# arnaucube/go-snark-study

Measured on AMD Instinct MI355X. Metric: Groth16 constraints/sec (prove) at 2^20 R1CS, higher is better.
Workload: dtype u32 (9x29-bit Montgomery limbs of the 254-bit BN128 fields)

## Files before the change

### go-snark-study_amd/capi.py

```python
import ctypes
import os
import threading

import numpy as np

_HERE = os.path.dirname(os.path.abspath(__file__))
_LIB = None
_LOCK = threading.Lock()
_INIT_DEVICE = None

u64p = ctypes.POINTER(ctypes.c_uint64)
u32p = ctypes.POINTER(ctypes.c_uint32)
intp = ctypes.POINTER(ctypes.c_int)
Handle = ctypes.c_uint64


class GosnarkHipError(RuntimeError):
    def __init__(self, code, msg):
        super().__init__("libgosnark_hip: status %d: %s" % (code, msg))
        self.code = code


class Timing(ctypes.Structure):
    _fields_ = ([(n, ctypes.c_float) for n in
                 ("total_ms", "plan_ms", "accumulate_ms", "reduce_ms", "poly_ms", "h2d_ms", "acc_g1_ms", "acc_g2_ms")]
                + [("acc_g1_launches", ctypes.c_uint32), ("acc_g2_launches", ctypes.c_uint32),
                   ("acc_g1_terms", ctypes.c_uint64), ("acc_g2_terms", ctypes.c_uint64),
                   ("acc_g1_adds", ctypes.c_uint64), ("acc_g2_adds", ctypes.c_uint64),
                   ("window_bits", ctypes.c_uint32), ("fallbacks", ctypes.c_uint32),
                   ("plan_digits", ctypes.c_uint64), ("plan_entries", ctypes.c_uint64), ("heavy_buckets", ctypes.c_uint32), ("reserved", ctypes.c_uint32)])


class Memory(ctypes.Structure):
    _fields_ = [(n, ctypes.c_uint64) for n in ("device_total_bytes", "device_free_bytes", "library_bytes", "object_bytes", "table_bytes",
                                               "workspace_bytes", "objects", "evictions")]


def lib_path():
    return os.environ.get("GS_LIB") or os.path.join(_HERE, "libgosnark_hip.so")


_SIGS = {
    "gs_init": [intp, ctypes.c_int],
    "gs_free": [Handle],
    "gs_len": [Handle, ctypes.POINTER(ctypes.c_size_t)],
    "gs_g1_upload": [u64p, ctypes.c_size_t, ctypes.POINTER(Handle)],
    "gs_g2_upload": [u64p, ctypes.c_size_t, ctypes.POINTER(Handle)],
    "gs_g1_download": [Handle, u64p, ctypes.c_size_t],
    "gs_g2_download": [Handle, u64p, ctypes.c_size_t],
    "gs_g1_fixed_base": [u64p, ctypes.c_size_t, ctypes.POINTER(Handle)],
    "gs_g2_fixed_base": [u64p, ctypes.c_size_t, ctypes.POINTER(Handle)],
    "gs_scalars_upload": [u64p, ctypes.c_size_t, ctypes.POINTER(Handle)],
    "gs_scalars_download": [Handle, u64p, ctypes.c_size_t],
    "gs_scalars_update": [Handle, u64p, ctypes.c_size_t],
    "gs_msm_g1": [Handle, u64p, ctypes.c_size_t, ctypes.c_size_t, u64p, intp],
    "gs_msm_g2": [Handle, u64p, ctypes.c_size_t, ctypes.c_size_t, u64p, intp],
    "gs_msm_g1_resident": [Handle, ctypes.c_size_t, Handle, ctypes.c_size_t, ctypes.c_size_t, u64p, intp],
    "gs_msm_g2_resident": [Handle, ctypes.c_size_t, Handle, ctypes.c_size_t, ctypes.c_size_t, u64p, intp],
    "gs_msm_g1_begin": [Handle, ctypes.c_size_t, Handle, ctypes.c_size_t, ctypes.c_size_t, u64p],
    "gs_msm_g2_begin": [Handle, ctypes.c_size_t, Handle, ctypes.c_size_t, ctypes.c_size_t, u64p],
    "gs_msm_end": [ctypes.c_uint64, u64p, intp],
    "gs_g1_sum_affine": [u64p, intp, ctypes.c_size_t, u64p, intp],
    "gs_g2_sum_affine": [u64p, intp, ctypes.c_size_t, u64p, intp],
    "gs_poly_mul": [u64p, ctypes.c_size_t, u64p, ctypes.c_size_t, u64p],
    "gs_poly_div": [u64p, ctypes.c_size_t, u64p, ctypes.c_size_t, u64p, u64p],
    "gs_poly_add": [u64p, ctypes.c_size_t, u64p, ctypes.c_size_t, u64p],
    "gs_poly_sub": [u64p, ctypes.c_size_t, u64p, ctypes.c_size_t, u64p],
    "gs_poly_eval": [u64p, ctypes.c_size_t, u64p, u64p],
    "gs_lagrange_interpolation": [u64p, ctypes.c_size_t, u64p],
    "gs_zpoly": [ctypes.c_size_t, u64p],
    "gs_r1cs_to_px": [ctypes.c_size_t, ctypes.c_size_t, u32p, u32p, u64p, u32p, u32p, u64p, u32p, u32p, u64p,
                      u64p, u64p, u64p, u64p, u64p],
    "gs_r1cs_upload": [ctypes.c_size_t, ctypes.c_size_t, u32p, u32p, u64p, u32p, u32p, u64p, u32p, u32p, u64p, ctypes.POINTER(Handle)],
    "gs_r1cs_px": [Handle, Handle, ctypes.POINTER(Handle)],
    "gs_groth16_pk_create": [Handle, Handle, Handle, Handle, Handle, u64p, u64p, u64p, u64p, u64p,
                             u64p, ctypes.c_size_t, ctypes.c_size_t, ctypes.c_size_t, ctypes.POINTER(Handle)],
    "gs_groth16_prove": [Handle, u64p, ctypes.c_size_t, u64p, ctypes.c_size_t, u64p, u64p, u64p, intp],
    "gs_groth16_prove_resident": [Handle, Handle, Handle, u64p, u64p, u64p, intp],
    "gs_groth16_prove_r1cs": [Handle, Handle, Handle, ctypes.POINTER(Handle), u64p, u64p, u64p, intp],
    "gs_groth16_prove_witness": [Handle, Handle, Handle, u64p, u64p, u64p, intp],
    "gs_groth16_prove_witness_begin": [Handle, Handle, Handle, u64p, u64p, u64p],
    "gs_groth16_pk_set_eval": [Handle, Handle],
    "gs_pk_eval_count": [Handle, ctypes.POINTER(ctypes.c_size_t)],
    "gs_pinocchio_pk_set_eval": [Handle, Handle],
    "gs_pinocchio_prove_witness_begin": [Handle, Handle, Handle, u64p],
    "gs_groth16_prove_begin": [Handle, Handle, Handle, u64p, u64p, u64p],
    "gs_groth16_prove_end": [ctypes.c_uint64, u64p, intp],
    "gs_groth16_prove_host_begin": [Handle, u64p, ctypes.c_size_t, u64p, ctypes.c_size_t, u64p, u64p, u64p],
    "gs_groth16_prove_witness_host_begin": [Handle, Handle, u64p, ctypes.c_size_t, u64p, u64p, u64p],
    "gs_groth16_prove_witness_host": [Handle, Handle, u64p, ctypes.c_size_t, u64p, u64p, u64p, intp],
    "gs_pinocchio_prove_host_begin": [Handle, u64p, ctypes.c_size_t, u64p, ctypes.c_size_t, u64p],
    "gs_pinocchio_prove_witness_host_begin": [Handle, Handle, u64p, ctypes.c_size_t, u64p],
    "gs_pinocchio_prove_witness_host": [Handle, Handle, u64p, ctypes.c_size_t, u64p, intp],
    "gs_ticket_cancel": [ctypes.c_uint64],
    "gs_groth16_pk_create_shard": [Handle, Handle, Handle, Handle, Handle, u64p, u64p, u64p, u64p, u64p, u64p, ctypes.c_size_t,
                                   ctypes.c_size_t, ctypes.c_size_t, ctypes.c_size_t, ctypes.c_size_t, ctypes.c_size_t, ctypes.POINTER(Handle)],
    "gs_groth16_pk_shard": [Handle, ctypes.c_size_t, ctypes.c_size_t, ctypes.POINTER(Handle)],
    "gs_groth16_prove_partials": [Handle, Handle, Handle, ctypes.c_size_t, ctypes.c_size_t, u64p, intp],
    "gs_groth16_finish": [Handle, u64p, intp, u64p, u64p, u64p, intp],
    "gs_groth16_setup": [ctypes.c_size_t, ctypes.c_size_t, ctypes.c_size_t, u32p, u32p, u64p, u32p, u32p, u64p, u32p, u32p, u64p,
                         u64p, ctypes.POINTER(Handle), u64p],
    "gs_groth16_pk_export": [Handle, ctypes.c_int, u64p, ctypes.c_size_t],
    "gs_pinocchio_setup": [ctypes.c_size_t, ctypes.c_size_t, ctypes.c_size_t, u32p, u32p, u64p, u32p, u32p, u64p, u32p, u32p, u64p,
                           u64p, ctypes.POINTER(Handle), u64p],
    "gs_pinocchio_pk_export": [Handle, ctypes.c_int, u64p, ctypes.c_size_t],
    "gs_pinocchio_pk_create": [Handle, Handle, Handle, Handle, Handle, Handle, Handle, Handle, u64p,
                               ctypes.c_size_t, ctypes.c_size_t, ctypes.c_size_t, ctypes.POINTER(Handle)],
    "gs_pinocchio_prove": [Handle, u64p, ctypes.c_size_t, u64p, ctypes.c_size_t, u64p, intp],
    "gs_pinocchio_prove_resident": [Handle, Handle, Handle, u64p, intp],
    "gs_pinocchio_prove_witness": [Handle, Handle, Handle, u64p, intp],
    "gs_pinocchio_prove_begin": [Handle, Handle, Handle, u64p],
    "gs_pinocchio_prove_end": [ctypes.c_uint64, u64p, intp],
    "gs_device_count": [],
    "gs_set_device": [ctypes.c_int],
    "gs_get_device": [],
    "gs_handle_device": [Handle],
    "gs_scalars_clone": [Handle, ctypes.c_size_t, ctypes.c_size_t, ctypes.c_int, ctypes.POINTER(Handle)],
    "gs_g1_clone": [Handle, ctypes.c_size_t, ctypes.c_size_t, ctypes.c_int, ctypes.POINTER(Handle)],
    "gs_g2_clone": [Handle, ctypes.c_size_t, ctypes.c_size_t, ctypes.c_int, ctypes.POINTER(Handle)],
    "gs_groth16_pk_shard_to": [Handle, ctypes.c_size_t, ctypes.c_size_t, ctypes.c_int, ctypes.POINTER(Handle)],
    "gs_comm_unique_id": [ctypes.POINTER(ctypes.c_uint8)],
    "gs_comm_init_rank": [ctypes.POINTER(ctypes.c_uint8), ctypes.c_int, ctypes.c_int],
    "gs_comm_init_local": [],
    "gs_comm_info": [intp, intp, intp, u64p],
    "gs_comm_allgather": [ctypes.c_void_p, ctypes.c_size_t, ctypes.c_void_p],
    "gs_msm_g1_multi": [ctypes.POINTER(Handle), ctypes.POINTER(Handle), ctypes.c_int, u64p, intp, intp],
    "gs_msm_g2_multi": [ctypes.POINTER(Handle), ctypes.POINTER(Handle), ctypes.c_int, u64p, intp, intp],
    "gs_groth16_prove_multi": [ctypes.POINTER(Handle), ctypes.POINTER(Handle), ctypes.POINTER(Handle), ctypes.c_int, u64p, u64p, u64p, intp, intp],
    "gs_groth16_prove_sharded": [Handle, Handle, Handle, u64p, u64p, u64p, intp],
    "gs_groth16_witness_values": [Handle, Handle, Handle, ctypes.POINTER(Handle), ctypes.POINTER(ctypes.c_uint32)],
    "gs_groth16_prove_partials_values": [Handle, Handle, Handle, ctypes.c_size_t, ctypes.c_size_t, u64p, intp],
    "gs_groth16_partials_values_begin": [Handle, Handle, Handle, ctypes.c_size_t, ctypes.c_size_t, u64p],
    "gs_groth16_partials_end": [ctypes.c_uint64, u64p, intp],
    "gs_groth16_prove_multi_values": [ctypes.POINTER(Handle), ctypes.POINTER(Handle), ctypes.POINTER(Handle), ctypes.c_int, u64p, u64p, u64p, intp, intp],
    "gs_groth16_prove_sharded_values": [Handle, Handle, Handle, u64p, u64p, u64p, intp],
    "gs_scalars_scatter": [Handle, ctypes.c_size_t, ctypes.c_int, ctypes.POINTER(Handle)],
    "gs_msm_g1_sharded": [Handle, Handle, u64p, intp],
    "gs_msm_g2_sharded": [Handle, Handle, u64p, intp],
    "gs_groth16_prove_batch": [ctypes.POINTER(Handle), ctypes.c_int, ctypes.POINTER(Handle), ctypes.POINTER(Handle), ctypes.c_size_t,
                               u64p, u64p, u64p, intp],
    "gs_pinocchio_pk_shard": [Handle, ctypes.c_size_t, ctypes.c_size_t, ctypes.POINTER(Handle)],
    "gs_pinocchio_pk_shard_to": [Handle, ctypes.c_size_t, ctypes.c_size_t, ctypes.c_int, ctypes.POINTER(Handle)],
    "gs_pinocchio_prove_partials": [Handle, Handle, Handle, ctypes.c_size_t, ctypes.c_size_t, u64p, intp],
    "gs_pinocchio_witness_values": [Handle, Handle, Handle, ctypes.POINTER(Handle), ctypes.POINTER(ctypes.c_uint32)],
    "gs_pinocchio_prove_partials_values": [Handle, Handle, Handle, ctypes.c_size_t, ctypes.c_size_t, u64p, intp],
    "gs_pinocchio_combine": [u64p, intp, ctypes.c_size_t, u64p, intp],
    "gs_pinocchio_prove_multi": [ctypes.POINTER(Handle), ctypes.POINTER(Handle), ctypes.POINTER(Handle), ctypes.c_int, u64p, intp, intp],
    "gs_pinocchio_prove_multi_values": [ctypes.POINTER(Handle), ctypes.POINTER(Handle), ctypes.POINTER(Handle), ctypes.c_int, u64p, intp, intp],
    "gs_pinocchio_prove_sharded": [Handle, Handle, Handle, u64p, intp],
    "gs_pinocchio_prove_sharded_values": [Handle, Handle, Handle, u64p, intp],
    "gs_pinocchio_prove_batch": [ctypes.POINTER(Handle), ctypes.c_int, ctypes.POINTER(Handle), ctypes.POINTER(Handle), ctypes.c_size_t, u64p, intp],
    "gs_last_timing": [ctypes.POINTER(Timing)],
    "gs_device_timing": [ctypes.c_int, ctypes.POINTER(Timing)],
    "gs_set_window_bits": [ctypes.c_int],
    "gs_set_eval_basis": [ctypes.c_int],
    "gs_memory_query": [ctypes.POINTER(Memory)],
    "gs_handle_bytes": [Handle, u64p, u64p],
    "gs_release_tables": [Handle],
    "gs_set_table_policy": [ctypes.c_int],
    "gs_build_tables": [Handle, ctypes.c_int],
    "gs_set_memory_limit": [ctypes.c_uint64],
    "gs_alloc_counters": [u64p, u64p],
    "gs_abi_sizes": [ctypes.POINTER(ctypes.c_size_t), ctypes.POINTER(ctypes.c_size_t)],
    "gs_trim": [],
    "gs_verify_set_strict": [ctypes.c_int],
    "gs_pairing": [u64p, u64p, u64p],
    "gs_pairing_check": [u64p, u64p, ctypes.c_size_t, intp],
    "gs_groth16_verify": [u64p, u64p, u64p, u64p, u64p, ctypes.c_size_t, u64p, ctypes.c_size_t, u64p, u64p, u64p, intp],
    "gs_pinocchio_verify": [u64p, u64p, u64p, u64p, u64p, u64p, u64p, u64p, ctypes.c_size_t, u64p, ctypes.c_size_t, u64p, intp, intp],
}
EXPORTS = sorted(list(_SIGS) + ["gs_shutdown", "gs_last_error", "gs_version", "gs_comm_destroy"])


def load_library():
    global _LIB
    with _LOCK:
        if _LIB is not None:
            return _LIB
        path = lib_path()
        try:
            import torch
        except ImportError:
            pass
        if not os.path.exists(path):
            raise GosnarkHipError(-1, "%s not found: build it with __graft_entry__.build() "
                                  "(hipcc --offload-arch=gfx950); there is no CPU fallback" % path)
        lib = ctypes.CDLL(path)
        missing = [n for n in EXPORTS if not hasattr(lib, n)]
        if missing:
            raise GosnarkHipError(-1, "%s lacks symbols declared in include/gosnark_hip.h: %s" % (path, missing))
        for name, args in _SIGS.items():
            fn = getattr(lib, name)
            fn.argtypes = args
            fn.restype = ctypes.c_int
        lib.gs_last_error.restype = ctypes.c_char_p
        lib.gs_version.restype = ctypes.c_char_p
        lib.gs_shutdown.restype = None
        lib.gs_comm_destroy.restype = None
        tb, mb = ctypes.c_size_t(0), ctypes.c_size_t(0)
        lib.gs_abi_sizes(ctypes.byref(tb), ctypes.byref(mb))
        if tb.value != ctypes.sizeof(Timing) or mb.value != ctypes.sizeof(Memory):
            raise GosnarkHipError(-1, "%s writes gs_timing / gs_memory of %d / %d bytes, this binding expects %d / %d: rebuild the library"
                                  % (path, tb.value, mb.value, ctypes.sizeof(Timing), ctypes.sizeof(Memory)))
        _LIB = lib
        return lib


def check(status):
# ... 219 lines not shown
def memory_query():
    init()
    m = Memory()
    check(load_library().gs_memory_query(ctypes.byref(m)))
    return {n: int(getattr(m, n)) for n, _ in Memory._fields_ if n != "reserved"}


def handle_bytes(h):
    a, b = ctypes.c_uint64(0), ctypes.c_uint64(0)
    check(load_library().gs_handle_bytes(Handle(_raw(h)), ctypes.cast(ctypes.byref(a), u64p), ctypes.cast(ctypes.byref(b), u64p)))
    return int(a.value), int(b.value)


def release_tables(h):
    check(load_library().gs_release_tables(Handle(_raw(h))))


TABLE_POLICY = {"auto": 0, "always": 1, "never": 2}


def set_table_policy(policy):
    init()
    check(load_library().gs_set_table_policy(TABLE_POLICY[policy] if isinstance(policy, str) else int(policy)))


def build_tables(h, route=0):
    check(load_library().gs_build_tables(Handle(_raw(h)), int(route)))


def set_memory_limit(nbytes):
    check(load_library().gs_set_memory_limit(ctypes.c_uint64(int(nbytes))))


def alloc_counters():
    a, b = ctypes.c_uint64(0), ctypes.c_uint64(0)
    check(load_library().gs_alloc_counters(ctypes.cast(ctypes.byref(a), u64p), ctypes.cast(ctypes.byref(b), u64p)))
    return int(a.value), int(b.value)


def scalars_update(handle, s_u64):
    a = np.ascontiguousarray(s_u64, dtype=np.uint64).reshape(-1, 4)
    check(load_library().gs_scalars_update(Handle(_raw(handle)), ptr64(a), a.shape[0]))


def trim():
    check(load_library().gs_trim())


def set_eval_basis(on):
    init()
    check(load_library().gs_set_eval_basis(1 if on else 0))


def set_window_bits(c):
    init()
    check(load_library().gs_set_window_bits(int(c)))


def zpoly(deg):
    init()
    out = np.zeros((deg + 1, 4), dtype=np.uint64)
    check(load_library().gs_zpoly(deg, ptr64(out)))
    return out


def msm_begin(bases, scalars, n, off=0, soff=0, g2=False):
    t = ctypes.c_uint64(0)
    fn = load_library().gs_msm_g2_begin if g2 else load_library().gs_msm_g1_begin
    check(fn(Handle(bases.h), off, Handle(scalars.h), soff, n, ctypes.cast(ctypes.byref(t), u64p)))
    return (t.value, g2)


def ticket_cancel(ticket):
    check(load_library().gs_ticket_cancel(ctypes.c_uint64(ticket[0] if isinstance(ticket, tuple) else ticket)))


def msm_end(ticket):
    t, g2 = ticket
    out = np.zeros(16 if g2 else 8, dtype=np.uint64)
    inf = ctypes.c_int(0)
    check(load_library().gs_msm_end(ctypes.c_uint64(t), ptr64(out), ctypes.byref(inf)))
    return _affine_result(out, inf, g2)


def _clone(fname, handle, off, n, target):
    h = Handle(0)
    check(getattr(load_library(), fname)(Handle(handle.h), off, n, int(target), ctypes.byref(h)))
    return DeviceHandle(h.value)


def scalars_clone(handle, target, off=0, n=None):
    return _clone("gs_scalars_clone", handle, off, len(handle) - off if n is None else n, target)


def g1_clone(handle, target, off=0, n=None):
    return _clone("gs_g1_clone", handle, off, len(handle) - off if n is None else n, target)


def g2_clone(handle, target, off=0, n=None):
    return _clone("gs_g2_clone", handle, off, len(handle) - off if n is None else n, target)


def scalars_scatter(full_handle, total, root, slice_handle=None):
    h = Handle(slice_handle.h if slice_handle is not None else 0)
    check(load_library().gs_scalars_scatter(Handle(full_handle.h if full_handle is not None else 0), int(total), int(root), ctypes.byref(h)))
    return slice_handle if slice_handle is not None else DeviceHandle(h.value)
# ... 60 lines not shown
```

### go-snark-study_amd/csrc/capi_msm.hip

```cpp
#include <algorithm>
#include <cstdlib>
#include <vector>

#include "msm.h"
#include "hostcopy.h"
#include "point_io.h"
#include "poly.h"
#include "prove.h"
#include "runtime.h"

using namespace gs;

namespace gs { void multi_shutdown(); }

namespace {


template <class T>
int upload_bases(Ctx& c, Kind kind, const uint64_t* jac, size_t n, gs_handle* out) {
  if (!out || (n && !jac)) return fail(GS_ERR_ARG, "null argument");
  if (n >= (1ull << 31)) return fail(GS_ERR_ARG, "too many points");
  constexpr size_t cw = T::kWords;
  auto b = std::make_unique<Bases>(kind);
  b->n = n;
// ... 500 lines not shown
  return guarded([&](Ctx& c) -> int {
    if (!out) return fail(GS_ERR_ARG, "null");
    *out = c.timing;
    return GS_OK;
  }, true, true);
}

int gs_device_timing(int logical_device, gs_timing* out) {
  if (!out) return fail(GS_ERR_ARG, "null");
  std::shared_ptr<Ctx> pc = ctx_ref(logical_device);
  if (!pc) return fail(GS_ERR_ARG, "gs_device_timing: no logical device %d", logical_device);
  Ctx& c = *pc;
  std::lock_guard<FairMutex> lk(c.mu);
  if (!c.ready) return fail(GS_ERR_NOT_INIT, "the library was shut down");
  *out = c.timing;
  return GS_OK;
}

int gs_ticket_cancel(uint64_t ticket) {
  return guarded([&](Ctx& c) -> int {
    for (int p = 0; p < Ctx::kMaxInFlight; ++p)
      if (c.inflight[p] && c.inflight[p]->ticket == ticket) {
        c.drain();
        c.inflight[p].reset();
        return GS_OK;
      }
    return fail(GS_ERR_ARG, "gs_ticket_cancel: unknown ticket %llu", (unsigned long long)ticket);
  }, true, true, ticket);
}

int gs_set_window_bits(int cbits) {
  if (cbits != 0 && (cbits < 8 || cbits > kMaxWindowBits)) return fail(GS_ERR_ARG, "window bits must be 0 (auto) or 8..%d", kMaxWindowBits);
  Registry& r = registry();
  std::lock_guard<std::mutex> rl(r.mu);
  if (r.ctxs.empty()) return fail(GS_ERR_NOT_INIT, "gs_init has not been called (or failed)");
  for (auto& pc : r.ctxs) {
    std::lock_guard<FairMutex> lk(pc->mu);
    pc->window_bits = cbits;
  }
  return GS_OK;
}

int gs_set_eval_basis(int enabled) {
  Registry& r = registry();
  std::lock_guard<std::mutex> rl(r.mu);
  if (r.ctxs.empty()) return fail(GS_ERR_NOT_INIT, "gs_init has not been called (or failed)");
  for (auto& pc : r.ctxs) {
    std::lock_guard<FairMutex> lk(pc->mu);
    pc->eval_basis = enabled != 0;
  }
  return GS_OK;
}

}
```

### go-snark-study_amd/csrc/capi_poly.hip

```cpp
#include "prove.h"

#include <algorithm>

using namespace gs;

extern "C" {

int gs_poly_mul(const uint64_t* a, size_t na, const uint64_t* b, size_t nb, uint64_t* out) {
  return guarded([&](Ctx& c) -> int {
    if (!a || !b || !out || na == 0 || nb == 0) return fail(GS_ERR_ARG, "gs_poly_mul: empty or null operand");
    if (na + nb > (1ull << 27)) return fail(GS_ERR_ARG, "gs_poly_mul: product too large");
    const uint32_t* da = upload_tmp(c, prove_state(c).up_a, a, na);
    const uint32_t* db = upload_tmp(c, prove_state(c).up_b, b, nb);
    const size_t nr = na + nb - 1;
    prove_state(c).up_o.ensure(nr * 32);
    poly_mul_dev(c, da, na, Form::Std, db, nb, Form::Std, prove_state(c).up_o.as<uint32_t>());
    poly_canon_dev(c, prove_state(c).up_o.as<uint32_t>(), nr, 0);
    download(c, out, prove_state(c).up_o.p, nr);
    return GS_OK;
  });
}

int gs_poly_div(const uint64_t* a, size_t na, const uint64_t* b, size_t nb, uint64_t* quo, uint64_t* rem) {
  return guarded([&](Ctx& c) -> int {
    if (!a || !b || !quo || nb == 0 || na < nb) return fail(GS_ERR_ARG, "gs_poly_div: need len(a) >= len(b) >= 1");
    bool lead_zero = true;
    for (int i = 0; i < 4; ++i) lead_zero = lead_zero && b[4 * (nb - 1) + i] == 0;
    if (lead_zero) return fail(GS_ERR_ARG, "gs_poly_div: leading coefficient of the divisor is zero");
    const uint32_t* da = upload_tmp(c, prove_state(c).up_a, a, na);
    const uint32_t* db = upload_tmp(c, prove_state(c).up_b, b, nb);
    Divisor d;
    divisor_init(c, d, db, nb);
    const size_t nq = na - nb + 1;
    prove_state(c).up_o.ensure((nq + na + nb) * 32);
    uint32_t* q = prove_state(c).up_o.as<uint32_t>();
    poly_quotient_dev(c, d, da, na, q);
    if (rem && nb > 1) {
      uint32_t* qb = q + nq * 8;
      poly_mul_dev(c, q, nq, Form::Std, db, nb, Form::Std, qb);
      uint32_t* rr = qb + (nq + nb - 1) * 8;
      poly_addsub_dev(c, da, nb - 1, qb, nb - 1, true, rr);
      poly_canon_dev(c, rr, nb - 1, 0);
      GS_HIP(hipMemcpyAsync(rem, rr, (nb - 1) * 32, hipMemcpyDeviceToHost, c.stream));
      GS_HIP(hipStreamSynchronize(c.stream));
    }
    poly_canon_dev(c, q, nq, 0);
    download(c, quo, q, nq);
    return GS_OK;
  });
}

static int addsub_api(const uint64_t* a, size_t na, const uint64_t* b, size_t nb, uint64_t* out, bool sub) {
  return guarded([&](Ctx& c) -> int {
    if ((na && !a) || (nb && !b) || !out) return fail(GS_ERR_ARG, "null operand");
    const size_t n = std::max(na, nb);
    if (n == 0) return GS_OK;
    const uint32_t* da = upload_tmp(c, prove_state(c).up_a, a, na);
    const uint32_t* db = upload_tmp(c, prove_state(c).up_b, b, nb);
    prove_state(c).up_o.ensure(n * 32);
    poly_addsub_dev(c, da, na, db, nb, sub, prove_state(c).up_o.as<uint32_t>());
    poly_canon_dev(c, prove_state(c).up_o.as<uint32_t>(), n, 0);
    download(c, out, prove_state(c).up_o.p, n);
    return GS_OK;
  });
}
int gs_poly_add(const uint64_t* a, size_t na, const uint64_t* b, size_t nb, uint64_t* out) { return addsub_api(a, na, b, nb, out, false); }
int gs_poly_sub(const uint64_t* a, size_t na, const uint64_t* b, size_t nb, uint64_t* out) { return addsub_api(a, na, b, nb, out, true); }

int gs_poly_eval(const uint64_t* v, size_t n, const uint64_t x[4], uint64_t out[4]) {
  return guarded([&](Ctx& c) -> int {
    if ((n && !v) || !x || !out) return fail(GS_ERR_ARG, "null operand");
    const uint32_t* dv = upload_tmp(c, prove_state(c).up_a, v, n);
    prove_state(c).up_o.ensure(32);
    poly_eval_dev(c, dv, n, x, prove_state(c).up_o.as<uint32_t>());
    download(c, out, prove_state(c).up_o.p, 1);
    return GS_OK;
  });
}

int gs_lagrange_interpolation(const uint64_t* values, size_t n, uint64_t* coeffs) {
  return guarded([&](Ctx& c) -> int {
    if (n == 0) return GS_OK;
    if (!values || !coeffs) return fail(GS_ERR_ARG, "gs_lagrange_interpolation: null argument");
    if (n >= (1ull << 26)) return fail(GS_ERR_ARG, "gs_lagrange_interpolation: too many nodes");
    const uint32_t* dv = upload_tmp(c, prove_state(c).up_a, values, n);
    prove_state(c).up_o.ensure(n * 32);
    interpolate_dev(c, dv, n, 1, prove_state(c).up_o.as<uint32_t>());
    poly_canon_dev(c, prove_state(c).up_o.as<uint32_t>(), n, 0);
    download(c, coeffs, prove_state(c).up_o.p, n);
    return GS_OK;
  });
}

int gs_zpoly(size_t deg, uint64_t* out) {
  return guarded([&](Ctx& c) -> int {
    if (!out) return fail(GS_ERR_ARG, "gs_zpoly: null output");
    if (deg >= (1ull << 26)) return fail(GS_ERR_ARG, "gs_zpoly: degree too large");
    prove_state(c).up_o.ensure((deg + 1) * 32);
    zpoly_dev(c, deg, prove_state(c).up_o.as<uint32_t>());
    download(c, out, prove_state(c).up_o.p, deg + 1);
// ... 6 lines not shown
```

### go-snark-study_amd/csrc/msm.hip

```cpp
#include "msm.h"
#include "hostcopy.h"

#include <algorithm>
#include <cmath>
#include <cstdlib>
#include <future>
#include <type_traits>

#include "msm_kernels.h"

namespace gs {

static_assert(sizeof(G1Xyzz) == PointIO<FqTag>::kXyzzWords * 4, "G1 XYZZ must be raw limbs");
static_assert(sizeof(G2Xyzz) == PointIO<Fq2Tag>::kXyzzWords * 4, "G2 XYZZ must be raw limbs");

static inline dim3 grid1(size_t n, int block = 256) { return dim3((unsigned)((n + block - 1) / block)); }

int choose_window_bits(uint32_t n, int forced) {
  if (forced >= 8 && forced <= kMaxWindowBits) return forced;
  static const double per_bucket = dev_knob_f("GS_WINDOW_COST_BUCKET", 6.0, 0.0, 64.0);
  static const int auto_max = (int)dev_knob("GS_AUTO_MAX_C", 17, 8, kMaxWindowBits);
  int best = 8;
  double best_cost = 1e300;
  for (int c = 8; c <= std::min(kMaxWindowBits, std::max(8, auto_max)); ++c) {
// ... 36 lines not shown
};
static MsmState& msm_state(Ctx& c) { return c.state<MsmState>(c.msm_state); }

static uint32_t choose_chunk(uint64_t entries, uint32_t nbuckets, const std::vector<LaunchShape>& users) {
  static const int forced = (int)dev_knob("GS_CHUNK", 0, 4, 1024, 4);
  if (forced >= 4 && forced % 4 == 0) return (uint32_t)forced;
  static const int forced_h = (int)dev_knob("GS_CHUNK_H", 0, 4, 1024, 4);
  if (forced_h && users.size() == 1 && users[0].njobs == 1 && !users[0].g2) return (uint32_t)forced_h;
  uint32_t chunk = entries >= (1ull << 27) ? 64u : entries >= (1ull << 23) ? 32u : 16u;
  while (chunk < 1024u && entries / std::max<uint32_t>(nbuckets, 1u) > 32ull * chunk) chunk *= 2;
  return chunk;
}

static uint32_t part_min_ranges() {
  static const uint32_t v = (uint32_t)dev_knob("GS_PART_MIN_R", 4, 2, 64);
  return v;
}
bool plan_partitions_first(int cbits) {
  if (cbits < 1) return false;
  return std::max<uint32_t>(1u, (1u << (cbits - 1)) >> kRangeLog) >= part_min_ranges();
}

uint32_t finite_mask_dev(Ctx& c, const uint32_t* g1_pts, const uint32_t* g2_pts, uint32_t n, uint32_t* mask_dev) {
  const size_t words = ((size_t)n + 31) / 32;
  GS_HIP(hipMemsetAsync(mask_dev, 0, std::max<size_t>(words, 1) * 4, c.stream));
  DevBuf cnt(4);
  GS_HIP(hipMemsetAsync(cnt.p, 0, 4, c.stream));
  if (n) hipLaunchKernelGGL(k_finite_mask, grid1(n), dim3(256), 0, c.stream, g1_pts, (uint32_t)PointIO<FqTag>::kAffineWords, g2_pts,
                            (uint32_t)PointIO<Fq2Tag>::kAffineWords, n, mask_dev, cnt.as<uint32_t>());
  GS_HIP(hipGetLastError());
  uint32_t host = 0;
  GS_HIP(hipMemcpyAsync(&host, cnt.p, 4, hipMemcpyDeviceToHost, c.stream));
  GS_HIP(hipStreamSynchronize(c.stream));
  return host;
}

void build_plan(Ctx& c, int slot, const uint32_t* scalars_dev, uint32_t n, MsmPlan& plan, const std::vector<LaunchShape>& users, int cbits,
                bool table_free, const uint32_t* term_index, uint32_t index_bias) {
  MsmState& ms = msm_state(c);
  PlanBuffers& pb = ms.plan_slots[slot % (3 * Ctx::kSlots)];
  plan.n = n;
  plan.table_free = table_free;
  plan.c = cbits ? cbits : (table_free ? choose_window_bits_free(n, c.window_bits) : choose_window_bits(n, c.window_bits));
  if (table_free && (plan.c < kMinFreeWindowBits || plan.c > kMaxFreeWindowBits))
    throw HipError{hipErrorInvalidValue, "table-free plan outside 9..16 window bits", __LINE__};
  plan.W = 254 / plan.c + 1;
  plan.B = 1u << (plan.c - 1);
  plan.nbuckets = table_free ? (uint32_t)plan.W * plan.B : plan.B;
  plan.chunk = choose_chunk((uint64_t)n * plan.W, plan.nbuckets, users);
  plan.maxchunks = (uint32_t)(((size_t)n * plan.W + plan.chunk - 1) / plan.chunk) + 1;
  const size_t ncount = (size_t)plan.nbuckets + 1;
  PlanParams pp{};
  pp.n = n; pp.c = plan.c; pp.W = plan.W; pp.B = plan.B;
  pp.R = std::max<uint32_t>(1u, plan.B >> kRangeLog);
  pp.tf = table_free ? 1u : 0u;
  {
    const uint32_t want = std::max<uint32_t>(1u, 256u / (plan.W * pp.R));
    const uint32_t by_size = std::max<uint32_t>(1u, (n + 16383u) / 16384u);
    const uint32_t by_mem = std::max<uint32_t>(1u, (uint32_t)((64ull << 20) / ((uint64_t)plan.B * plan.W * 4)));
    pp.S = std::max<uint32_t>(1u, std::min(std::min<uint32_t>(16u, std::max<uint32_t>(want, 1u)), std::min(by_size, by_mem)));
    if (pp.R == 1 && !table_free) pp.S = std::max<uint32_t>(1u, std::min<uint32_t>(16u, by_size));
  }
  pp.slice = (n + pp.S - 1) / pp.S;
  pp.stride = (n + 63u) & ~63u;
  const bool wide = plan_partitions_first(plan.c);
  if (wide && term_index) throw HipError{hipErrorInvalidValue, "plans over a term list cannot be sorted partition-first (plan_partitions_first)", __LINE__};
  const uint32_t nparts = (uint32_t)plan.W * pp.R;
  if (wide && nparts > kMaxParts) throw HipError{hipErrorInvalidValue, "too many (window, range) partitions", __LINE__};
  if (!wide) pb.digits.ensure((size_t)std::max<uint32_t>(pp.stride, 64u) * plan.W * sizeof(digit_t));
  else {
    pb.recs.ensure(std::max<size_t>((size_t)n * plan.W, 1) * 8);
    pb.parts.ensure((size_t)(3 * kMaxParts + 4) * 4);
  }
  pb.hist.ensure((size_t)plan.B * plan.W * pp.S * 4);
  pb.totals.ensure(ncount * 4);
  pb.offsets.ensure(ncount * 4);
  pb.entries.ensure(((size_t)plan.maxchunks + 1) * plan.chunk * 4);
  pb.chunk_bucket.ensure((size_t)plan.maxchunks * 4);
  pb.heavy_list.ensure((size_t)plan.nbuckets * 4);
  pb.counters.ensure(16);
  const size_t lds = (size_t)std::min<uint32_t>(plan.B, kRangeBuckets) * 4;
  static const int sort_block = (int)dev_knob("GS_SORT_BLOCK", kSortBlock, 64, kSortBlock, 64);
  if (!ms.lds_attr_set) {
    GS_HIP(hipFuncSetAttribute(reinterpret_cast<const void*>(k_hist), hipFuncAttributeMaxDynamicSharedMemorySize, 128 * 1024));
    GS_HIP(hipFuncSetAttribute(reinterpret_cast<const void*>(k_scatter), hipFuncAttributeMaxDynamicSharedMemorySize, 128 * 1024));
    GS_HIP(hipFuncSetAttribute(reinterpret_cast<const void*>(k_hist_part), hipFuncAttributeMaxDynamicSharedMemorySize, 128 * 1024));
    GS_HIP(hipFuncSetAttribute(reinterpret_cast<const void*>(k_scatter_part), hipFuncAttributeMaxDynamicSharedMemorySize, 128 * 1024));
    ms.lds_attr_set = true;
  }
  GS_HIP(hipMemsetAsync(pb.totals.as<uint32_t>() + plan.nbuckets, 0, 4, c.stream));
  GS_HIP(hipMemsetAsync(pb.counters.p, 0, 16, c.stream));
  uint32_t* part_count = pb.parts.as<uint32_t>();
  uint32_t* part_base = part_count ? part_count + kMaxParts : nullptr;
  uint32_t* part_cursor = part_count ? part_base + kMaxParts + 4 : nullptr;
  if (n > 0 && wide) {
    GS_HIP(hipMemsetAsync(part_count, 0, (size_t)nparts * 4, c.stream));
    hipLaunchKernelGGL(k_part_count, grid1(n, kPartBlock), dim3(kPartBlock), 0, c.stream, scalars_dev, pp, part_count);
    hipLaunchKernelGGL(k_part_scan, dim3(1), dim3(64), 0, c.stream, part_count, nparts, part_base, part_cursor);
    hipLaunchKernelGGL(k_part_scatter, grid1(n, kPartBlock * kPartPerThread), dim3(kPartBlock), 0, c.stream, scalars_dev, pp, part_base, part_cursor,
                       pb.recs.as<uint2>());
    hipLaunchKernelGGL(k_hist_part, dim3(8 * pp.S * ((nparts + 7) / 8)), dim3(sort_block), lds, c.stream, pb.recs.as<uint2>(), part_base, pp, pb.hist.as<uint32_t>());
    hipLaunchKernelGGL(k_colscan, grid1(plan.B), dim3(256), 0, c.stream, pb.hist.as<uint32_t>(), pp, pb.totals.as<uint32_t>());
  } else if (n > 0) {
    hipLaunchKernelGGL(k_digits, grid1(n), dim3(256), 0, c.stream, scalars_dev, pp, pb.digits.as<digit_t>(), term_index, index_bias);
    hipLaunchKernelGGL(k_hist, dim3(plan.W, pp.S, pp.R), dim3(sort_block), lds, c.stream, pb.digits.as<digit_t>(), pp, pb.hist.as<uint32_t>());
    if (table_free) hipLaunchKernelGGL(k_colscan_windows, grid1(plan.nbuckets), dim3(256), 0, c.stream, pb.hist.as<uint32_t>(), pp, pb.totals.as<uint32_t>());
    else hipLaunchKernelGGL(k_colscan, grid1(plan.B), dim3(256), 0, c.stream, pb.hist.as<uint32_t>(), pp, pb.totals.as<uint32_t>());
  } else {
    GS_HIP(hipMemsetAsync(pb.totals.p, 0, ncount * 4, c.stream));
  }
  exclusive_scan(c, pb, pb.totals.as<uint32_t>(), pb.offsets.as<uint32_t>(), (uint32_t)ncount);
  if (n > 0) {
    if (wide) hipLaunchKernelGGL(k_scatter_part, dim3(8 * pp.S * ((nparts + 7) / 8)), dim3(sort_block), lds, c.stream, pb.recs.as<uint2>(), part_base, pp,
                                 pb.hist.as<uint32_t>(), pb.offsets.as<uint32_t>(), pb.entries.as<uint32_t>());
    else hipLaunchKernelGGL(k_scatter, dim3(plan.W, pp.S, pp.R), dim3(sort_block), lds, c.stream, pb.digits.as<digit_t>(), pp, pb.hist.as<uint32_t>(),
                            pb.offsets.as<uint32_t>(), pb.entries.as<uint32_t>(), term_index, index_bias);
    hipLaunchKernelGGL(k_chunk_map, grid1(plan.nbuckets), dim3(256), 0, c.stream, pb.offsets.as<uint32_t>(), plan.nbuckets, plan.chunk,
                       pb.chunk_bucket.as<uint32_t>(), pb.heavy_list.as<uint32_t>(), pb.counters.as<uint32_t>());
  }
  GS_HIP(hipGetLastError());
  plan.offsets = pb.offsets.as<uint32_t>();
  plan.entries = pb.entries.as<uint32_t>();
  plan.chunk_bucket = pb.chunk_bucket.as<uint32_t>();
  plan.heavy_list = pb.heavy_list.as<uint32_t>();
  plan.heavy_count = pb.counters.as<uint32_t>();
}

template <class T>
static void enqueue_table_slabs(hipStream_t stream, DevBuf& scratch, const uint32_t* src, size_t n, int cbits, DevBuf& rows, size_t first, size_t last,
                                size_t slab) {
  const int W = 254 / cbits + 1;
  if (first >= last) return;
  static const bool per_row = dev_flag("GS_TABLE_PER_ROW");
  if (per_row || W <= 2) {
    if (first == 0) hipLaunchKernelGGL(k_build_table<T>, grid1(n), dim3(256), 0, stream, src, (uint32_t)n, cbits, W, rows.as<uint32_t>());
  } else {
    constexpr size_t sw = PointIO<T>::kXyzzWords + PointIO<T>::kXyzzWords / 4;
    slab = std::min<size_t>(std::max<size_t>(slab, 1), n);
    scratch.ensure(slab * (size_t)(W - 1) * sw * 4);
    for (size_t at = first; at < last; at += slab) {
      const size_t count = std::min(slab, last - at);
      hipLaunchKernelGGL(k_build_table_batched<T>, grid1(count), dim3(256), 0, stream, src, (uint32_t)n, (uint32_t)at, (uint32_t)count, cbits, W,
                         rows.as<uint32_t>(), scratch.as<uint32_t>());
    }
  }
  GS_HIP(hipGetLastError());
}
template <class T>
static void enqueue_table_build(Ctx& c, hipStream_t stream, DevBuf& scratch, const uint32_t* src, size_t n, int cbits, DevBuf& fresh,
                                size_t slab_max = (size_t)1 << 18) {
  constexpr size_t aw = PointIO<T>::kAffineWords;
  const int W = 254 / cbits + 1;
  fresh.alloc(std::max<size_t>(n, 1) * W * aw * 4);
  enqueue_table_slabs<T>(stream, scratch, src, n, cbits, fresh, 0, n, slab_max);
}

template <class T>
static void ensure_table(Ctx& c, BaseTable& t, const uint32_t* row0, size_t n, int cbits) {
  if (t.c == cbits && t.n == n && t.rows.p) return;
  table_settle(c, t, false);
  const uint32_t* src = row0 ? row0 : t.rows.as<uint32_t>();
  if (!src || (!row0 && t.n != n)) throw HipError{hipErrorInvalidValue, "window table rebuild without its points", __LINE__};
  DevBuf fresh;
  enqueue_table_build<T>(c, c.stream, msm_state(c).table_scratch, src, n, cbits, fresh);
  GS_HIP(hipStreamSynchronize(c.stream));
  t.rows = std::move(fresh);
  t.n = n; t.c = cbits; t.W = 254 / cbits + 1;
  t.uses = 0;
// ... 457 lines not shown
```

### go-snark-study_amd/csrc/msm_kernels.h

```cpp
#pragma once
#include <hip/hip_runtime.h>
#include <stdint.h>

#include "ec.h"
#include "point_io.h"

namespace gs {

struct PlanParams {
  uint32_t n;
  int c;
  int W;
  uint32_t B;
  uint32_t S;
  uint32_t slice;
  uint32_t stride;
  uint32_t R;
  uint32_t tf;
};
constexpr uint32_t kRangeLog = 15;
constexpr uint32_t kRangeBuckets = 1u << kRangeLog;

GS_HD int32_t next_digit(const uint32_t (&k)[8], const PlanParams& pp, int w, uint32_t& carry) {
  uint32_t raw = scalar_bits(k, w * pp.c, pp.c) + carry;
  if (raw > pp.B) { carry = 1; return (int32_t)raw - (int32_t)(2u * pp.B); }
  carry = 0;
  return (int32_t)raw;
}

using digit_t = uint32_t;
__global__ void __launch_bounds__(256) k_digits(const uint32_t* __restrict__ scalars, PlanParams pp, digit_t* __restrict__ digits,
                                                 const uint32_t* __restrict__ term_index, uint32_t index_bias) {
  wave_priority<GS_PRIO_PLAN>();
  const uint32_t i = blockIdx.x * blockDim.x + threadIdx.x;
  if (i >= pp.n) return;
  const uint32_t src = term_index ? term_index[i] - index_bias : i;
  uint32_t k[8];
  const uint4* s4 = reinterpret_cast<const uint4*>(scalars + (size_t)src * 8);
  uint4 lo = s4[0], hi = s4[1];
  k[0] = lo.x; k[1] = lo.y; k[2] = lo.z; k[3] = lo.w; k[4] = hi.x; k[5] = hi.y; k[6] = hi.z; k[7] = hi.w;
  scalar_canon(k);
  uint32_t carry = 0;
  for (int w = 0; w < pp.W; ++w) {
    const int32_t d = next_digit(k, pp, w, carry);
    digits[(size_t)w * pp.stride + i] = (digit_t)(d + (int32_t)pp.B - 1);
  }
}

__global__ void __launch_bounds__(256) k_finite_mask(const uint32_t* __restrict__ a, uint32_t wa, const uint32_t* __restrict__ b, uint32_t wb, uint32_t n,
                                                      uint32_t* __restrict__ mask, uint32_t* __restrict__ count) {
  const uint32_t i = blockIdx.x * blockDim.x + threadIdx.x;
  bool finite = false;
  if (i < n) {
    uint32_t acc = 0;
    if (a) for (uint32_t k = 0; k < wa; ++k) acc |= a[(size_t)i * wa + k];
    if (b) for (uint32_t k = 0; k < wb; ++k) acc |= b[(size_t)i * wb + k];
    finite = acc != 0;
  }
  if (finite) { atomicOr(&mask[i >> 5], 1u << (i & 31u)); atomicAdd(count, 1u); }
}

constexpr int kSortBlock = 1024;

__global__ void __launch_bounds__(kSortBlock) k_hist(const digit_t* __restrict__ digits, PlanParams pp, uint32_t* __restrict__ hist) {
  wave_priority<GS_PRIO_PLAN>();
  extern __shared__ uint32_t sh[];
  const uint32_t w = blockIdx.x, s = blockIdx.y, r = blockIdx.z;
  const uint32_t nb = min(pp.B, kRangeBuckets), base = r << kRangeLog;
  for (uint32_t b = threadIdx.x; b < nb; b += blockDim.x) sh[b] = 0;
  __syncthreads();
  const uint32_t lo = s * pp.slice, hi = min(pp.n, lo + pp.slice);
  const digit_t* row = digits + (size_t)w * pp.stride;
  const int32_t zero = (int32_t)pp.B - 1;
  for (uint32_t i = lo + threadIdx.x; i < hi; i += blockDim.x) {
    const int32_t d = (int32_t)row[i] - zero;
    if (d != 0) {
      const uint32_t b = (uint32_t)(d < 0 ? -d : d) - 1u;
      if ((b >> kRangeLog) == r) atomicAdd(&sh[b - base], 1u);
    }
  }
  __syncthreads();
  uint32_t* out = hist + ((size_t)w * pp.S + s) * pp.B + base;
  for (uint32_t b = threadIdx.x; b < nb; b += blockDim.x) out[b] = sh[b];
}

__global__ void __launch_bounds__(256) k_colscan(uint32_t* __restrict__ hist, PlanParams pp, uint32_t* __restrict__ totals) {
  wave_priority<GS_PRIO_PLAN>();
  const uint32_t b = blockIdx.x * blockDim.x + threadIdx.x;
  if (b >= pp.B) return;
  uint32_t* col = hist + b;
  const uint32_t nq = (uint32_t)pp.W * pp.S;
  uint32_t run = 0;
  for (uint32_t q = 0; q < nq; ++q) { const uint32_t t = col[(size_t)q * pp.B]; col[(size_t)q * pp.B] = run; run += t; }
  totals[b] = run;
}

__global__ void __launch_bounds__(256) k_colscan_windows(uint32_t* __restrict__ hist, PlanParams pp, uint32_t* __restrict__ totals) {
  wave_priority<GS_PRIO_PLAN>();
  const uint32_t i = blockIdx.x * blockDim.x + threadIdx.x;
  if (i >= (uint32_t)pp.W * pp.B) return;
  const uint32_t w = i / pp.B, b = i % pp.B;
  uint32_t* col = hist + (size_t)w * pp.S * pp.B + b;
  uint32_t run = 0;
  for (uint32_t q = 0; q < pp.S; ++q) { const uint32_t t = col[(size_t)q * pp.B]; col[(size_t)q * pp.B] = run; run += t; }
  totals[i] = run;
}

__global__ void __launch_bounds__(kSortBlock) k_scatter(const digit_t* __restrict__ digits, PlanParams pp, const uint32_t* __restrict__ hist,
                                                         const uint32_t* __restrict__ offsets, uint32_t* __restrict__ entries,
                                                         const uint32_t* __restrict__ term_index, uint32_t index_bias) {
  wave_priority<GS_PRIO_PLAN>();
  extern __shared__ uint32_t sh[];
  const uint32_t w = blockIdx.x, s = blockIdx.y, r = blockIdx.z;
  const uint32_t nb = min(pp.B, kRangeBuckets), base = r << kRangeLog;
  const uint32_t* pre = hist + ((size_t)w * pp.S + s) * pp.B + base;
  const uint32_t* off = offsets + (pp.tf ? (size_t)w * pp.B : (size_t)0);
  for (uint32_t b = threadIdx.x; b < nb; b += blockDim.x) sh[b] = off[base + b] + pre[b];
  __syncthreads();
  const uint32_t lo = s * pp.slice, hi = min(pp.n, lo + pp.slice);
  const digit_t* row = digits + (size_t)w * pp.stride;
  const int32_t zero = (int32_t)pp.B - 1;
  for (uint32_t i = lo + threadIdx.x; i < hi; i += blockDim.x) {
    const int32_t d = (int32_t)row[i] - zero;
    if (d != 0) {
      const uint32_t b = (uint32_t)(d < 0 ? -d : d) - 1u;
      if ((b >> kRangeLog) == r) {
        const uint32_t pos = atomicAdd(&sh[b - base], 1u);
        const uint32_t id = term_index ? term_index[i] - index_bias : i;
        entries[pos] = id | (w << kWindowShift) | (d < 0 ? kSignBit : 0u);
      }
    }
  }
}

constexpr int kPartBlock = 256;
constexpr int kPartPerThread = 4;
constexpr uint32_t kMaxParts = 512;

GS_HD void load_scalar_canon(const uint32_t* __restrict__ scalars, uint32_t i, uint32_t (&k)[8]) {
  const uint4* s4 = reinterpret_cast<const uint4*>(scalars + (size_t)i * 8);
  const uint4 lo = s4[0], hi = s4[1];
  k[0] = lo.x; k[1] = lo.y; k[2] = lo.z; k[3] = lo.w; k[4] = hi.x; k[5] = hi.y; k[6] = hi.z; k[7] = hi.w;
  scalar_canon(k);
}

__global__ void __launch_bounds__(kPartBlock) k_part_count(const uint32_t* __restrict__ scalars, PlanParams pp, uint32_t* __restrict__ part_count) {
  wave_priority<GS_PRIO_PLAN>();
  __shared__ uint32_t cnt[kMaxParts];
  const uint32_t nparts = (uint32_t)pp.W * pp.R;
  for (uint32_t t = threadIdx.x; t < nparts; t += kPartBlock) cnt[t] = 0;
  __syncthreads();
  const uint32_t i = blockIdx.x * kPartBlock + threadIdx.x;
  if (i < pp.n) {
    uint32_t k[8];
    load_scalar_canon(scalars, i, k);
    uint32_t carry = 0;
    for (int w = 0; w < pp.W; ++w) {
      const int32_t d = next_digit(k, pp, w, carry);
      if (d != 0) atomicAdd(&cnt[(uint32_t)w * pp.R + (((uint32_t)(d < 0 ? -d : d) - 1u) >> kRangeLog)], 1u);
    }
  }
  __syncthreads();
  for (uint32_t t = threadIdx.x; t < nparts; t += kPartBlock) if (cnt[t]) atomicAdd(&part_count[t], cnt[t]);
}

__global__ void __launch_bounds__(64) k_part_scan(uint32_t* __restrict__ part_count, uint32_t nparts, uint32_t* __restrict__ part_base,
                                                    uint32_t* __restrict__ part_cursor) {
  wave_priority<GS_PRIO_PLAN>();
  if (blockIdx.x != 0 || threadIdx.x != 0) return;
  uint32_t run = 0;
  for (uint32_t t = 0; t < nparts; ++t) { part_base[t] = run; run += part_count[t]; part_cursor[t] = 0; part_count[t] = 0; }
  part_base[nparts] = run;
}

__global__ void __launch_bounds__(kPartBlock) k_part_scatter(const uint32_t* __restrict__ scalars, PlanParams pp, const uint32_t* __restrict__ part_base,
                                                              uint32_t* __restrict__ part_cursor, uint2* __restrict__ recs) {
  wave_priority<GS_PRIO_PLAN>();
  __shared__ uint32_t cnt[kMaxParts];
  const uint32_t nparts = (uint32_t)pp.W * pp.R;
  for (uint32_t t = threadIdx.x; t < nparts; t += kPartBlock) cnt[t] = 0;
// ... 628 lines not shown
```

### go-snark-study_amd/csrc/poly.h

```cpp
#pragma once
#include "fp29.h"
#include "runtime.h"

namespace gs {

enum class Form { Std, Mont };

int ceil_log2(size_t n);

void ntt_forward(Ctx& c, uint32_t* data, int logt, int logm);
void ntt_inverse_unscaled(Ctx& c, uint32_t* data, int logt, int logm);
void ntt_forward_n(Ctx& c, uint32_t* data, size_t total, int logm);
void ntt_inverse_unscaled_n(Ctx& c, uint32_t* data, size_t total, int logm);

void poly_mul_dev(Ctx& c, const uint32_t* a, size_t na, Form fa, const uint32_t* b, size_t nb, Form fb, uint32_t* out);

void poly_inv_series_dev(Ctx& c, const uint32_t* f_mont, size_t nf, size_t k, uint32_t* g_mont);

struct Divisor {
  size_t nb = 0;
  DevBuf b_std;
  size_t k = 0;
  DevBuf inv_rev_mont;
  int logn_spec = 0;
  size_t k_spec = 0;
  DevBuf inv_spec;
};
void divisor_init(Ctx& c, Divisor& d, const uint32_t* b_std_dev, size_t nb);
void poly_quotient_dev(Ctx& c, Divisor& d, const uint32_t* a_std, size_t na, uint32_t* quo_std);

void zpoly_dev(Ctx& c, size_t deg, uint32_t* out_std);

void interpolate_dev(Ctx& c, const uint32_t* values_std, size_t n, size_t nvec, uint32_t* coeffs_std);
bool hx_direct_dev(Ctx& c, const uint32_t* vals_std, size_t n, size_t dz, uint32_t* hx_out_std);
bool hx_values_dev(Ctx& c, const uint32_t* vals_std, size_t n, size_t dz, uint32_t* hv_out_std);
void r1cs_check_dev(Ctx& c, const uint32_t* vals_std, size_t n, size_t dz, uint32_t* bad_dev);
void hx_from_values_dev(Ctx& c, const uint32_t* hv_std, size_t n, size_t dz, uint32_t* hx_out_std);
void spmv_dev(Ctx& c, const uint32_t* rowptr, const uint32_t* col, const uint32_t* val_std, const uint32_t* x_mont, size_t nrows, size_t ncols,
              uint32_t* out_std);

void poly_addsub_dev(Ctx& c, const uint32_t* a, size_t na, const uint32_t* b, size_t nb, bool subtract, uint32_t* out);
void poly_canon_dev(Ctx& c, uint32_t* x, size_t n, int mode );
void poly_eval_dev(Ctx& c, const uint32_t* v_std, size_t n, const uint64_t x[4], uint32_t* out_dev);

Fe<ModR, 2> fr_from_words_mont(const uint64_t w[4]);
void fr_words_from_mont(const Fe<ModR, 2>& a, uint64_t out[4]);
void fr_mul_words(const uint64_t a[4], const uint64_t b[4], uint64_t out[4]);
void fr_inv_words(const uint64_t a[4], uint64_t out[4]);
void fr_sub_words(const uint64_t a[4], const uint64_t b[4], uint64_t out[4]);
bool fr_is_zero_words(const uint64_t a[4]);
void fr_falling_product_words(const uint64_t x[4], size_t count, uint64_t out[4]);

const uint32_t* interpolation_weights_dev(Ctx& c, size_t n);
void lagrange_at_dev(Ctx& c, size_t n, const uint64_t tau[4], const uint64_t mtau[4], uint32_t* out_mont);
void setup_scalars_dev(Ctx& c, const uint32_t* at, const uint32_t* bt, const uint32_t* ct, size_t m, size_t npublic, const uint64_t kalpha[4],
                       const uint64_t kbeta[4], const uint64_t inv_delta[4], const uint64_t inv_gamma[4], uint32_t* cd, uint32_t* ic);
void pinocchio_scalars_dev(Ctx& c, const uint32_t* at, const uint32_t* bt, const uint32_t* ct, size_t m, const uint64_t rhoa[4], const uint64_t rhob[4],
                           const uint64_t rhoc[4], const uint64_t ka[4], const uint64_t kb[4], const uint64_t kc[4], const uint64_t kbeta[4],
                           uint32_t* const out[7]);
void scaled_powers_dev(Ctx& c, const uint64_t base[4], const uint64_t scale_std[4], size_t count, uint32_t* out_std);
void scale_mont_by_std_dev(Ctx& c, const uint32_t* a_mont, const uint64_t scale_std[4], size_t n, uint32_t* out_std);

}
```

### go-snark-study_amd/csrc/poly.hip

```cpp
#include "poly.h"

#include <algorithm>
#include <vector>

#include "poly_kernels.h"

namespace gs {

static inline dim3 grid1(size_t n, int block = 256) { return dim3((unsigned)((n + block - 1) / block)); }

int ceil_log2(size_t n) {
  int l = 0;
  while (((size_t)1 << l) < n) ++l;
  return l;
}

static FrConst to_const(const Fe<ModR, 2>& a) {
  FrConst c;
  for (int i = 0; i < NL; ++i) c.l[i] = a.l[i];
  return c;
}
Fe<ModR, 2> fr_from_words_mont(const uint64_t w[4]) {
  uint32_t u[8];
  for (int i = 0; i < 4; ++i) { u[2 * i] = (uint32_t)w[i]; u[2 * i + 1] = (uint32_t)(w[i] >> 32); }
  return to_mont(unpack32<ModR>(u));
}
static Fe<ModR, 2> fr_small_mont(uint64_t v) {
  uint64_t w[4] = {v, 0, 0, 0};
  return fr_from_words_mont(w);
}

struct Twiddles {
  int logn = 0;
  DevBuf fwd, inv;
};
struct NodeTree {
  size_t n = 0, total = 0, pad = 0;
  int L = 0;
  std::vector<DevBuf> mspec;
  DevBuf root;
  DevBuf weights;
  uint64_t stamp = 0;
};

struct PolyState {
  Twiddles tw;
  DevBuf ws_a, ws_b, ws_c, ws_d;
  NodeTree trees[2];
  uint64_t tree_clock = 0;
  DevBuf cur_a, cur_b, wide, nxt;
  DevBuf long_rows;
  size_t fact_top = 0;
  DevBuf fact, invfact;
  struct HxTables {
    size_t n = 0, dz = 0, N = 0;
    uint64_t stamp = 0;
    DevBuf inv_spec, shift_spec, t1, t2;
  };
  static constexpr int kHxSlots = 4;
  HxTables hx[kHxSlots];
  uint64_t hx_clock = 0;
  DevBuf hx_conv, hx_hv, hx_g, hx_bad;
};
static PolyState& poly_state(Ctx& c) { return c.state<PolyState>(c.poly_state); }

static Twiddles& ensure_twiddles(Ctx& c, int logn) {
  Twiddles& tw = poly_state(c).tw;
  if (logn <= tw.logn) return tw;
  if (logn > ModR::kTwoAdicity) throw HipError{hipErrorInvalidValue, "NTT size exceeds the 2-adicity of Fr (2^28)", __LINE__};
  logn = std::max(logn, 16);
  const uint32_t half = 1u << (logn - 1);
  Fe<ModR, 2> w, wi;
  for (int i = 0; i < NL; ++i) { w.l[i] = ModR::omega28_mont(i); wi.l[i] = ModR::omega28_inv_mont(i); }
  for (int i = 0; i < ModR::kTwoAdicity - logn; ++i) { w = sqr(w); wi = sqr(wi); }
  tw.fwd.alloc((size_t)half * kTwWords * 4);
  tw.inv.alloc((size_t)half * kTwWords * 4);
  hipLaunchKernelGGL(k_twiddle_gen, grid1(half), dim3(256), 0, c.stream, tw.fwd.as<uint32_t>(), half, to_const(w));
  hipLaunchKernelGGL(k_twiddle_gen, grid1(half), dim3(256), 0, c.stream, tw.inv.as<uint32_t>(), half, to_const(wi));
  GS_HIP(hipGetLastError());
  tw.logn = logn;
  return tw;
}

void ntt_forward(Ctx& c, uint32_t* data, int logt, int logm) { ntt_forward_n(c, data, (size_t)1 << logt, logm); }
void ntt_inverse_unscaled(Ctx& c, uint32_t* data, int logt, int logm) { ntt_inverse_unscaled_n(c, data, (size_t)1 << logt, logm); }

struct NttPass { int s_lo, k, clog; uint32_t ntiles; };
static std::vector<NttPass> ntt_schedule(size_t total, int logm) {
  std::vector<NttPass> v;
  const int low = std::min(kNttMaxStages, logm);
  int hi = logm;
  while (hi > low) {
    const int k = std::min(kNttMaxStages, hi - low);
    const int s_lo = hi - k;
    const int clog = std::min(kNttTileLog - k, s_lo);
    v.push_back(NttPass{s_lo, k, clog, (uint32_t)(total >> (k + clog))});
    hi = s_lo;
  }
  int clog = kNttTileLog - low;
  while (clog > 0 && ((total >> low) & (((size_t)1 << clog) - 1))) --clog;
  v.push_back(NttPass{0, low, clog, (uint32_t)(total >> (low + clog))});
  return v;
}

void ntt_forward_n(Ctx& c, uint32_t* data, size_t total, int logm) {
  if (logm == 0 || total == 0) return;
  Twiddles& tw = ensure_twiddles(c, logm);
  for (const NttPass& p : ntt_schedule(total, logm))
    hipLaunchKernelGGL((k_ntt_pass<false, kNttLoadPlain>), dim3(p.ntiles), dim3(256), 0, c.stream, data, tw.fwd.as<uint32_t>(), tw.logn, p.s_lo, p.k, p.clog, NttLoadAux{});
  GS_HIP(hipGetLastError());
}

void ntt_inverse_unscaled_n(Ctx& c, uint32_t* data, size_t total, int logm) {
  if (logm == 0 || total == 0) return;
  Twiddles& tw = ensure_twiddles(c, logm);
// ... 64 lines not shown
  uint32_t* A = poly_state(c).ws_a.as<uint32_t>();
  uint32_t* B = poly_state(c).ws_b.as<uint32_t>();
  copy_padded(c, a, na, A, N);
  copy_padded(c, b, nb, B, N);
  ntt_forward(c, A, logn, logn);
  ntt_forward(c, B, logn, logn);
  hipLaunchKernelGGL(k_pw_mul, grid1(N), dim3(256), 0, c.stream, A, B, A, (uint32_t)N);
  ntt_inverse_unscaled(c, A, logn, logn);
  hipLaunchKernelGGL(k_pw_mul_const, grid1(nr), dim3(256), 0, c.stream, A, inv_n_const(logn, extra), out, (uint32_t)nr);
  GS_HIP(hipGetLastError());
}

void poly_inv_series_dev(Ctx& c, const uint32_t* f, size_t nf, size_t k, uint32_t* g) {
  Fe<ModR, 6> f0v;
  uint32_t f0w[8];
  GS_HIP(hipMemcpyAsync(f0w, f, 32, hipMemcpyDeviceToHost, c.stream));
  GS_HIP(hipStreamSynchronize(c.stream));
  f0v = unpack32<ModR>(f0w);
  if (is_zero(f0v)) throw HipError{hipErrorInvalidValue, "series inverse of a polynomial with zero constant term", __LINE__};
  Fe<ModR, 2> g0 = inv(reduce2(f0v));
  uint32_t g0w[8];
  {
    Fe<ModR, 1> cg = canon(g0);
    pack32<ModR>(cg, g0w);
  }
  GS_HIP(hipMemcpyAsync(g, g0w, 32, hipMemcpyHostToDevice, c.stream));
  GS_HIP(hipStreamSynchronize(c.stream));
  const FrConst two = to_const(fr_small_mont(2));
  size_t t = 1;
  while (t < k) {
    const size_t t2 = std::min(2 * t, k);
    const size_t fl = std::min(nf, t2);
    poly_state(c).ws_c.ensure((std::max(fl, t2) + t) * 32);
    poly_state(c).ws_d.ensure((t2 + t) * 32);
    uint32_t* E = poly_state(c).ws_c.as<uint32_t>();
    uint32_t* U = poly_state(c).ws_d.as<uint32_t>();
    poly_mul_dev(c, f, fl, Form::Mont, g, t, Form::Mont, E);
    const size_t el = std::min(fl + t - 1, t2);
    hipLaunchKernelGGL(k_two_minus, grid1(t2), dim3(256), 0, c.stream, E, two, U, (uint32_t)el, (uint32_t)t2);
    poly_mul_dev(c, g, t, Form::Mont, U, t2, Form::Mont, E);
    GS_HIP(hipMemcpyAsync(g, E, t2 * 32, hipMemcpyDeviceToDevice, c.stream));
    t = t2;
  }
  GS_HIP(hipGetLastError());
}

void divisor_init(Ctx& c, Divisor& d, const uint32_t* b_std_dev, size_t nb) {
  d.nb = nb;
  d.b_std.alloc(nb * 32);
  GS_HIP(hipMemcpyAsync(d.b_std.p, b_std_dev, nb * 32, hipMemcpyDeviceToDevice, c.stream));
  d.k = 0;
  d.logn_spec = 0;
  d.k_spec = 0;
}

static void divisor_ensure(Ctx& c, Divisor& d, size_t k) {
  if (k <= d.k) return;
  const size_t fl = std::min(d.nb, k);
  DevBuf f(fl * 32);
  hipLaunchKernelGGL(k_copy_reversed, grid1(fl), dim3(256), 0, c.stream, d.b_std.as<uint32_t>(), (uint32_t)(d.nb - fl), (uint32_t)fl,
                     f.as<uint32_t>(), (uint32_t)fl);
  poly_canon_dev(c, f.as<uint32_t>(), fl, 1);
  d.inv_rev_mont.alloc(k * 32);
  poly_inv_series_dev(c, f.as<uint32_t>(), fl, k, d.inv_rev_mont.as<uint32_t>());
  GS_HIP(hipStreamSynchronize(c.stream));
  d.k = k;
  d.logn_spec = 0;
}

void poly_quotient_dev(Ctx& c, Divisor& d, const uint32_t* a, size_t na, uint32_t* quo) {
  if (na < d.nb) return;
  const size_t k = na - d.nb + 1;
  divisor_ensure(c, d, k);
  const int logn = ceil_log2(2 * k - 1);
  const size_t N = (size_t)1 << logn;
  if (d.logn_spec != logn || d.k_spec != k) {
    d.inv_spec.alloc(N * 32);
    copy_padded(c, d.inv_rev_mont.as<uint32_t>(), k, d.inv_spec.as<uint32_t>(), N);
    ntt_forward(c, d.inv_spec.as<uint32_t>(), logn, logn);
    d.logn_spec = logn;
    d.k_spec = k;
  }
  poly_state(c).ws_a.ensure(N * 32);
  uint32_t* A = poly_state(c).ws_a.as<uint32_t>();
  hipLaunchKernelGGL(k_copy_reversed, grid1(N), dim3(256), 0, c.stream, a, (uint32_t)(na - k), (uint32_t)k, A, (uint32_t)N);
  ntt_forward(c, A, logn, logn);
  if (logn >= 1) ntt_inverse_unscaled_of_product_n(c, A, N, logn, d.inv_spec.as<uint32_t>());
  else hipLaunchKernelGGL(k_pw_mul, grid1(N), dim3(256), 0, c.stream, A, d.inv_spec.as<uint32_t>(), A, (uint32_t)N);
  poly_state(c).ws_b.ensure(k * 32);
  hipLaunchKernelGGL(k_copy_reversed, grid1(k), dim3(256), 0, c.stream, A, 0u, (uint32_t)k, poly_state(c).ws_b.as<uint32_t>(), (uint32_t)k);
  hipLaunchKernelGGL(k_pw_mul_const, grid1(k), dim3(256), 0, c.stream, poly_state(c).ws_b.as<uint32_t>(), inv_n_const(logn, 0), quo, (uint32_t)k);
  GS_HIP(hipGetLastError());
}


static void prefix_products(Ctx& c, int mode, uint32_t top, uint32_t count, uint32_t* out, Fe<ModR, 2>* last_host) {
  const uint32_t ntiles = (count + kPpTile - 1) / kPpTile;
  DevBuf tiles((size_t)ntiles * 32);
  hipLaunchKernelGGL(k_pp_tiles, dim3(ntiles), dim3(kPpBlock), 0, c.stream, mode, top, count, out, tiles.as<uint32_t>());
  if (ntiles > 1) {
    hipLaunchKernelGGL(k_pp_tile_scan, dim3(1), dim3(1024), 0, c.stream, tiles.as<uint32_t>(), ntiles);
    hipLaunchKernelGGL(k_pp_apply, grid1(count), dim3(256), 0, c.stream, out, tiles.as<uint32_t>(), count);
  }
  GS_HIP(hipGetLastError());
  if (last_host) {
    uint32_t w[8];
    GS_HIP(hipMemcpyAsync(w, out + (size_t)(count - 1) * 8, 32, hipMemcpyDeviceToHost, c.stream));
    GS_HIP(hipStreamSynchronize(c.stream));
    *last_host = reduce2(unpack32<ModR>(w));
  }
  GS_HIP(hipStreamSynchronize(c.stream));
}
static void ensure_factorials(Ctx& c, size_t top) {
  PolyState& ps = poly_state(c);
  if (top <= ps.fact_top) return;
  top = std::max<size_t>(top, 2 * ps.fact_top);
  if (top >= (1ull << 31)) throw HipError{hipErrorInvalidValue, "factorial table too large", __LINE__};
  DevBuf fwd(top * 32), rev(top * 32);
  Fe<ModR, 2> top_fact;
  prefix_products(c, 0, (uint32_t)top, (uint32_t)top, fwd.as<uint32_t>(), &top_fact);
  prefix_products(c, 1, (uint32_t)top, (uint32_t)top, rev.as<uint32_t>(), nullptr);
  ps.fact.alloc((top + 1) * 32);
  ps.invfact.alloc((top + 1) * 32);
  hipLaunchKernelGGL(k_fact_tables, grid1(top + 1), dim3(256), 0, c.stream, fwd.as<uint32_t>(), rev.as<uint32_t>(), to_const(inv(top_fact)), (uint32_t)top,
                     ps.fact.as<uint32_t>(), ps.invfact.as<uint32_t>());
  GS_HIP(hipGetLastError());
  GS_HIP(hipStreamSynchronize(c.stream));
  ps.fact_top = top;
}

static void build_weights(Ctx& c, NodeTree& t) {
  ensure_factorials(c, std::max<size_t>(t.n, 1));
  t.weights.alloc(std::max<size_t>(t.n, 1) * 32);
  if (t.n) hipLaunchKernelGGL(k_bary_weights, grid1(t.n), dim3(256), 0, c.stream, poly_state(c).invfact.as<uint32_t>(), (uint32_t)t.n, t.weights.as<uint32_t>());
  GS_HIP(hipGetLastError());
  GS_HIP(hipStreamSynchronize(c.stream));
}

static NodeTree& ensure_tree(Ctx& c, size_t n, bool need_weights) {
  NodeTree* t = nullptr;
  PolyState& ps = poly_state(c);
  for (auto& x : ps.trees) if (x.n == n && x.root.p) t = &x;
  if (!t) {
    t = (ps.trees[0].stamp <= ps.trees[1].stamp) ? &ps.trees[0] : &ps.trees[1];
// ... 282 lines not shown
```

### go-snark-study_amd/csrc/poly_kernels.h

```cpp
#pragma once
#include <hip/hip_runtime.h>
#include <stdint.h>

#include "fp29.h"

namespace gs {

using Fr6 = Fe<ModR, 6>;
using Fr2 = Fe<ModR, 2>;

GS_HD Fr6 load_fr(const uint32_t* p) {
  const uint4* q = reinterpret_cast<const uint4*>(p);
  const uint4 lo = q[0], hi = q[1];
  uint32_t w[8] = {lo.x, lo.y, lo.z, lo.w, hi.x, hi.y, hi.z, hi.w};
  return unpack32<ModR>(w);
}
GS_HD void store_fr(uint32_t* p, const Fr2& a) {
  Fr2 x = a;
  carry_full(x);
  Fe<ModR, 1> y;
#pragma unroll
  for (int i = 0; i < NL; ++i) y.l[i] = x.l[i];
  uint32_t w[8];
  pack32<ModR>(y, w);
// ... 88 lines not shown
GS_HD void ntt_dif_butterfly(int step, Bfly (&x)[N], const Fe<ModR, 1> (&w)[N], bool trivial) {
  ntt_dif_step<16, N>(x, w, (step & 3) == 3, trivial);
}
template <int B, int N>
GS_HD void ntt_dit_step(Bfly (&x)[N], const Fe<ModR, 1> (&w)[N], bool lazy_in, bool lazy_out, bool trivial) {
  static_assert(N == 1 || N == 2, "one or two butterflies per thread");
  Fr2 t[N];
  if (trivial) {
#pragma unroll
    for (int k = 0; k < N; ++k)
#pragma unroll
      for (int l = 0; l < NL; ++l) t[k].l[l] = x[k].b[l];
  } else if (lazy_in) {
    Lz<ModR, B, 3> b[N];
#pragma unroll
    for (int k = 0; k < N; ++k)
#pragma unroll
      for (int l = 0; l < NL; ++l) b[k].l[l] = x[k].b[l];
    if constexpr (N == 2) dots2<ModR>(dot_of(b[0], w[0]), dot_of(b[1], w[1]), t[0], t[1]);
    else t[0] = mul_lazy(b[0], w[0]);
  } else {
    Fe<ModR, B> b[N];
#pragma unroll
    for (int k = 0; k < N; ++k)
#pragma unroll
      for (int l = 0; l < NL; ++l) b[k].l[l] = x[k].b[l];
    if constexpr (N == 2) dots2<ModR>(dot_of(b[0], w[0]), dot_of(b[1], w[1]), t[0], t[1]);
    else t[0] = mul_lazy(b[0], w[0]);
  }
#pragma unroll
  for (int k = 0; k < N; ++k) {
    uint32_t p[NL], m[NL];
#pragma unroll
    for (int l = 0; l < NL; ++l) { p[l] = x[k].a[l] + t[k].l[l]; m[l] = x[k].a[l] + (ModR::tbias(3, l) - t[k].l[l]); }
    static_assert(ModR::tbias_k(3) == 3, "the DIT bound table (B + 2, B + 3) assumes the 3r bias");
    if (!lazy_out) {
      Fe<ModR, B + 3> pp, mm;
#pragma unroll
      for (int l = 0; l < NL; ++l) { pp.l[l] = p[l]; mm.l[l] = m[l]; }
      carry_save(pp); carry_save(mm);
#pragma unroll
      for (int l = 0; l < NL; ++l) { p[l] = pp.l[l]; m[l] = mm.l[l]; }
    }
#pragma unroll
    for (int l = 0; l < NL; ++l) { x[k].a[l] = p[l]; x[k].b[l] = m[l]; }
  }
}
template <int N>
GS_HD void ntt_dit_butterfly(int step, int nsteps, Bfly (&x)[N], const Fe<ModR, 1> (&w)[N], bool trivial) {
  const bool lazy_out = (step & 1) == 0 && step + 1 < nsteps;
  ntt_dit_step<20, N>(x, w, true, lazy_out, trivial);
}

constexpr int kNttLoadPlain = 0, kNttLoadScaled = 1, kNttLoadWeighed = 2;
struct NttLoadAux {
  const uint32_t* aux0;
  const uint32_t* aux1;
  uint32_t n;
  uint32_t logN;
};

template <bool kInverse, int kLoad = kNttLoadPlain>
__global__ void __launch_bounds__(256) k_ntt_pass(uint32_t* __restrict__ x, const uint32_t* __restrict__ tw, int tw_logn, int s_lo, int k, int clog, NttLoadAux aux) {
  wave_priority<GS_PRIO_POLY>();
  __shared__ uint32_t sh[NL * kNttTile];
  const uint32_t R = 1u << k, C = 1u << clog, E = R << clog;
  const uint32_t tile = blockIdx.x;
  size_t base;
  uint32_t qstride, cstride;
  if (s_lo == 0) { base = (size_t)tile * E; qstride = 1; cstride = R; }
  else {
    const uint32_t chunks = (1u << s_lo) >> clog;
    const uint32_t hi = tile / chunks, lc = tile - hi * chunks;
    base = ((size_t)hi << (s_lo + k)) + ((size_t)lc << clog); qstride = 1u << s_lo; cstride = 1;
  }
  for (uint32_t e = threadIdx.x; e < E; e += 256) {
    uint32_t q, cc;
    if (s_lo == 0) { q = e & (R - 1); cc = e >> k; } else { cc = e & (C - 1); q = e >> clog; }
    const size_t gi = base + (size_t)q * qstride + (size_t)cc * cstride;
    Fr2 v;
    if constexpr (kLoad == kNttLoadWeighed) {
      const size_t vec = gi >> aux.logN;
      const uint32_t j = (uint32_t)(gi & (((size_t)1 << aux.logN) - 1));
      if (j < aux.n) v = mul(load_fr(aux.aux0 + (vec * aux.n + j) * 8), load_fr(aux.aux1 + (size_t)j * 8));
      else v = fe_zero<ModR, 2>();
    } else if constexpr (kLoad == kNttLoadScaled) {
      v = mul(reduce2(load_fr(x + gi * 8)), load_fr(aux.aux0 + (gi & (((size_t)1 << aux.logN) - 1)) * 8));
    } else {
      v = reduce2(load_fr(x + gi * 8));
    }
    const uint32_t le = (q << clog) + cc;
#pragma unroll
    for (int l = 0; l < NL; ++l) sh[l * kNttTile + le] = v.l[l];
  }
  __syncthreads();
  auto twiddle_at = [&](uint32_t q0, uint32_t cc, int b) {
    const size_t gi = base + (size_t)q0 * qstride + (size_t)cc * cstride;
    const int s = s_lo + b;
    const uint32_t j = (uint32_t)gi & ((1u << s) - 1u);
    return load_twiddle(tw + ((size_t)j << (tw_logn - 1 - s)) * kTwWords);
  };
  int step = 0;
  for (; step < k; ++step) {
    const int b = kInverse ? step : k - 1 - step;
    const bool trivial = (s_lo + b) == 0;
    auto slots = [&](uint32_t u, uint32_t& e0, uint32_t& e1, uint32_t& q0, uint32_t& cc) {
      cc = u & (C - 1);
      const uint32_t qq = u >> clog;
      q0 = ((qq >> b) << (b + 1)) | (qq & ((1u << b) - 1u));
      e0 = (q0 << clog) + cc; e1 = e0 + ((1u << b) << clog);
    };
    uint32_t u = threadIdx.x;
    for (; u + 256 < E / 2; u += 512) {
      uint32_t e0[2], e1[2], q0[2], cc[2];
      slots(u, e0[0], e1[0], q0[0], cc[0]);
      slots(u + 256, e0[1], e1[1], q0[1], cc[1]);
      Fe<ModR, 1> w[2];
      if (!trivial) { w[0] = twiddle_at(q0[0], cc[0], b); w[1] = twiddle_at(q0[1], cc[1], b); }
      Bfly x[2];
#pragma unroll
      for (int t = 0; t < 2; ++t)
#pragma unroll
        for (int l = 0; l < NL; ++l) { x[t].a[l] = sh[l * kNttTile + e0[t]]; x[t].b[l] = sh[l * kNttTile + e1[t]]; }
      if constexpr (kInverse) ntt_dit_butterfly<2>(step, k, x, w, trivial);
      else ntt_dif_butterfly<2>(step, x, w, trivial);
#pragma unroll
      for (int t = 0; t < 2; ++t)
#pragma unroll
        for (int l = 0; l < NL; ++l) { sh[l * kNttTile + e0[t]] = x[t].a[l]; sh[l * kNttTile + e1[t]] = x[t].b[l]; }
    }
    for (; u < E / 2; u += 256) {
      uint32_t e0, e1, q0, cc;
      slots(u, e0, e1, q0, cc);
      Fe<ModR, 1> w[1];
      if (!trivial) w[0] = twiddle_at(q0, cc, b);
      Bfly x[1];
#pragma unroll
      for (int l = 0; l < NL; ++l) { x[0].a[l] = sh[l * kNttTile + e0]; x[0].b[l] = sh[l * kNttTile + e1]; }
      if constexpr (kInverse) ntt_dit_butterfly<1>(step, k, x, w, trivial);
      else ntt_dif_butterfly<1>(step, x, w, trivial);
#pragma unroll
      for (int l = 0; l < NL; ++l) { sh[l * kNttTile + e0] = x[0].a[l]; sh[l * kNttTile + e1] = x[0].b[l]; }
    }
    __syncthreads();
  }
  for (uint32_t e = threadIdx.x; e < E; e += 256) {
    uint32_t q, cc;
    if (s_lo == 0) { q = e & (R - 1); cc = e >> k; } else { cc = e & (C - 1); q = e >> clog; }
    const uint32_t le = (q << clog) + cc;
    Fe<ModR, kNttEndBound> v;
#pragma unroll
    for (int l = 0; l < NL; ++l) v.l[l] = sh[l * kNttTile + le];
    store_fr(x + (base + (size_t)q * qstride + (size_t)cc * cstride) * 8, reduce2(v));
  }
}

__global__ void __launch_bounds__(256) k_pw_mul(const uint32_t* __restrict__ a, const uint32_t* __restrict__ b,
                                                 uint32_t* __restrict__ out, uint32_t n) {
  wave_priority<GS_PRIO_POLY>();
  const uint32_t i = blockIdx.x * blockDim.x + threadIdx.x;
  if (i >= n) return;
  store_fr(out + (size_t)i * 8, mul(load_fr(a + (size_t)i * 8), load_fr(b + (size_t)i * 8)));
}
__global__ void __launch_bounds__(256) k_pw_mul_const(const uint32_t* __restrict__ a, FrConst k, uint32_t* __restrict__ out, uint32_t n) {
  wave_priority<GS_PRIO_POLY>();
  const uint32_t i = blockIdx.x * blockDim.x + threadIdx.x;
  if (i >= n) return;
  store_fr(out + (size_t)i * 8, mul(load_fr(a + (size_t)i * 8), from_const(k)));
}
__global__ void __launch_bounds__(256) k_addsub(const uint32_t* __restrict__ a, uint32_t na, const uint32_t* __restrict__ b, uint32_t nb,
                                                 int subtract, uint32_t* __restrict__ out, uint32_t n) {
  const uint32_t i = blockIdx.x * blockDim.x + threadIdx.x;
  if (i >= n) return;
  const Fr6 x = (i < na) ? load_fr(a + (size_t)i * 8) : fe_zero<ModR, 6>();
  const Fr6 y = (i < nb) ? load_fr(b + (size_t)i * 8) : fe_zero<ModR, 6>();
  if (subtract) store_fr(out + (size_t)i * 8, reduce2(sub(x, y)));
  else store_fr(out + (size_t)i * 8, reduce2(add(x, y)));
}
__global__ void __launch_bounds__(256) k_copy_reversed(const uint32_t* __restrict__ src, uint32_t first, uint32_t count,
                                                        uint32_t* __restrict__ dst, uint32_t total) {
  wave_priority<GS_PRIO_POLY>();
  const uint32_t i = blockIdx.x * blockDim.x + threadIdx.x;
  if (i >= total) return;
  uint4* d = reinterpret_cast<uint4*>(dst + (size_t)i * 8);
  if (i < count) {
    const uint4* s = reinterpret_cast<const uint4*>(src + (size_t)(first + count - 1 - i) * 8);
    d[0] = s[0]; d[1] = s[1];
  } else {
    d[0] = make_uint4(0, 0, 0, 0); d[1] = d[0];
  }
}
__global__ void __launch_bounds__(256) k_convert(uint32_t* __restrict__ x, uint32_t n, int mode) {
  const uint32_t i = blockIdx.x * blockDim.x + threadIdx.x;
  if (i >= n) return;
  const Fr6 v = load_fr(x + (size_t)i * 8);
  if (mode == 1) store_fr_canon(x + (size_t)i * 8, canon(to_mont(v)));
  else if (mode == 2) store_fr_canon(x + (size_t)i * 8, from_mont(v));
  else store_fr_canon(x + (size_t)i * 8, canon(v));
}
__global__ void __launch_bounds__(256) k_two_minus(const uint32_t* __restrict__ e, FrConst two, uint32_t* __restrict__ out, uint32_t n, uint32_t total) {
  const uint32_t i = blockIdx.x * blockDim.x + threadIdx.x;
  if (i >= total) return;
  if (i >= n) { store_fr(out + (size_t)i * 8, fe_zero<ModR, 2>()); return; }
  const Fr6 v = load_fr(e + (size_t)i * 8);
  if (i == 0) store_fr(out, reduce2(sub(from_const(two), v)));
  else store_fr(out + (size_t)i * 8, reduce2(neg(v)));
}

__global__ void __launch_bounds__(256) k_zp_leaves(uint32_t* __restrict__ out, uint32_t deg, uint32_t total) {
  const uint32_t i = blockIdx.x * blockDim.x + threadIdx.x;
  if (i >= total) return;
  if (i >= deg) { store_fr(out + (size_t)i * 8, fe_zero<ModR, 2>()); return; }
  uint32_t w[8] = {i + 1u, 0, 0, 0, 0, 0, 0, 0};
  store_fr_canon(out + (size_t)i * 8, canon(neg(to_mont(unpack32<ModR>(w)))));
}
__global__ void __launch_bounds__(256) k_expand_blocks(const uint32_t* __restrict__ src, uint32_t* __restrict__ dst, uint32_t d, uint32_t total2) {
// ... 368 lines not shown
```

### go-snark-study_amd/csrc/prove.hip

```cpp
#include "prove.h"

#include <algorithm>
#include <cstdlib>
#include <cstring>
#include <functional>
#include <chrono>
#include <future>
#include <vector>

#include "hostcopy.h"
#include "point_io.h"

using namespace gs;

const uint32_t* gs::upload_tmp(Ctx& c, DevBuf& buf, const uint64_t* host, size_t n) {
  buf.ensure(std::max<size_t>(n, 1) * 32);
  if (n) {
    PhaseTimer th(c.stream);
    staged_h2d(c, buf.p, host, n * 32, c.stream);
    th.stop();
    c.timing.h2d_ms += th.ms();
  }
  return buf.as<uint32_t>();
}
void gs::download(Ctx& c, uint64_t* host, const void* dev, size_t n) {
  if (n) GS_HIP(hipMemcpyAsync(host, dev, n * 32, hipMemcpyDeviceToHost, c.stream));
  GS_HIP(hipStreamSynchronize(c.stream));
}

namespace {

constexpr size_t kG1Aff = 16, kG2Aff = 32;

void copy_points(Ctx& c, const Bases* b, size_t words, DevBuf& dst) {
  dst.alloc(std::max<size_t>(b->n, 1) * words * 4);
  if (b->n) GS_HIP(hipMemcpyAsync(dst.p, b->buf.p, b->n * words * 4, hipMemcpyDeviceToDevice, c.stream));
}

struct DevScalars {
  const uint32_t* p;
  size_t n;
  const uint64_t* host = nullptr;
  hipStream_t host_stream = nullptr;
  hipEvent_t host_done = nullptr;
  std::function<void(Ctx&)> produce;
  std::function<bool(Ctx&, uint32_t*)> produce_hx;
  std::function<void(Ctx&, uint32_t*, uint32_t*)> produce_hv;
  const uint32_t* hv_slice = nullptr;
};
DevScalars resident(const Scalars* s) { return DevScalars{s->buf.as<uint32_t>(), s->n}; }

size_t quotient_len(size_t npx, size_t nz) { return npx >= nz ? npx - nz + 1 : 0; }
constexpr int kRetryExact = 1;


struct ProofSums {
  std::vector<G1Xyzz> g1w;
  G2Xyzz g2w;
  G1Xyzz h;
};

struct Shard { size_t index = 0, count = 1; };
static void shard_range(size_t n, const Shard& sh, size_t& lo, size_t& hi) {
  const size_t q = n / sh.count, rem = n % sh.count;
  lo = sh.index * q + std::min(sh.index, rem);
  hi = lo + q + (sh.index < rem ? 1 : 0);
}

static long host_stage_mode() {
  static const long mode = run_knob("GS_HOST_STAGE", 1, 0, 2);
  return mode;
}
struct ProofStreams {
  hipStream_t planw = nullptr, poly = nullptr, tail_g2 = nullptr, tail_g1 = nullptr;
  bool poly_first = false;
};
static ProofStreams proof_streams(Ctx& c, bool pipelined, size_t nterms, bool from_witness, int parity) {
  static const long mode = run_knob("GS_PLANW_STREAM", 1, 0, 2);
  static const long slot_mode = run_knob("GS_SLOT_STREAMS", 0, 0, 1);
  if (pipelined) c.next_tails((uint32_t)nterms);
  ProofStreams ps;
  if (pipelined && slot_mode == 1 && parity >= 0 && parity < Ctx::kAuxStreams && c.aux_stream[parity] != c.main_stream) {
    ps.planw = ps.poly = ps.tail_g2 = ps.tail_g1 = c.aux_stream[parity];
    ps.poly_first = true;
    return ps;
  }
  const bool own = pipelined && c.aux_stream[2] != c.aux_stream[1] &&
                   (mode == 2 || (mode == 1 && nterms >= ((size_t)1 << 19) && (from_witness || nterms >= ((size_t)1 << 21))));
  ps.poly = c.aux_stream[1];
  ps.planw = own ? c.aux_stream[2] : c.aux_stream[1];
  ps.tail_g2 = own ? c.aux_stream[0] : c.tail_stream(0);
  ps.tail_g1 = own ? c.aux_stream[0] : c.tail_stream(1);
  return ps;
}

struct HostInputs {
  hipEvent_t w_done = nullptr, px_done = nullptr;
  std::shared_ptr<PhaseTimer> th2d;
  void create() {
    if (!w_done) GS_HIP(hipEventCreateWithFlags(&w_done, hipEventDisableTiming));
    if (!px_done) GS_HIP(hipEventCreateWithFlags(&px_done, hipEventDisableTiming));
  }
  ~HostInputs() { for (hipEvent_t e : {w_done, px_done}) if (e) (void)hipEventDestroy(e); }
};

static const uint32_t* term_list_range(const DevBuf& index_dev, const std::vector<uint32_t>& index_host, size_t base, size_t nterms, uint32_t& count) {
  const auto lo = std::lower_bound(index_host.begin(), index_host.end(), (uint32_t)base);
  const auto hi = std::lower_bound(lo, index_host.end(), (uint32_t)(base + nterms));
  count = (uint32_t)(hi - lo);
  return index_dev.as<uint32_t>() + (lo - index_host.begin());
}

struct ProofInFlight : InFlightBase {
  ProverKey* pk = nullptr;
  ProofStreams streams;
  HostInputs in;
  hipEvent_t planw = nullptr, planh = nullptr, done_main = nullptr, done_g2 = nullptr, done_g1w = nullptr, done_h = nullptr;
  bool split_b = false;
  hipEvent_t planb = nullptr, done_g1b = nullptr;
  MsmPending pend_g1b;
  std::shared_ptr<PhaseTimer> tplanb;
  std::unique_ptr<PhaseTimer> total;
  MsmPending pend_g1w, pend_g2w, pend_h;
  std::shared_ptr<PhaseTimer> tpoly, tplanw, tplanh;
  const uint32_t* bad_host = nullptr;
  std::function<int(Ctx&, ProofSums&)> exact_route;
  std::function<void(const std::vector<G1Xyzz>&)> on_g1w;
  ProofInFlight() {
    for (hipEvent_t* e : {&planw, &planh, &done_main, &done_g2, &done_g1w, &done_h, &planb, &done_g1b}) GS_HIP(hipEventCreateWithFlags(e, hipEventDisableTiming));
  }
  void wait_device() const override {
    for (hipEvent_t e : {done_g2, done_g1w, done_h, done_main}) if (e) GS_HIP(hipEventSynchronize(e));
    if (split_b && done_g1b) GS_HIP(hipEventSynchronize(done_g1b));
  }
  ~ProofInFlight() override {
    for (hipEvent_t e : {planw, planh, done_main, done_g2, done_g1w, done_h, planb, done_g1b}) if (e) (void)hipEventDestroy(e);
  }
};

static long split_b_percent() {
  static const long pct = run_knob("GS_SPLIT_B_PERCENT", 55, 0, 100);
  return pct;
}

int proof_enqueue(Ctx& c, ProverKey* pk, DevScalars w, DevScalars px, const Shard& shard, int parity, bool wait_inputs, bool pipelined,
                  ProofInFlight& st) {
  DevBuf& hxbuf = prove_state(c).hx[parity];
  if (w.n != pk->nvars) return fail(GS_ERR_SHAPE, "len(w) = %zu but the key has %zu variables", w.n, pk->nvars);
  const bool eval = (bool)px.produce_hv || px.hv_slice;
  const size_t nh = eval ? pk->n_eval : quotient_len(px.n, pk->nz);
  if (!eval && nh > pk->len_h) return fail(GS_ERR_SHAPE, pk->hx_too_long, nh, pk->len_h);
  const bool sliced = pk->shard_count > 1;
  if (sliced && (shard.index != pk->shard_index || shard.count != pk->shard_count))
    return fail(GS_ERR_ARG, "this key holds shard %zu of %zu of the term ranges only: call gs_%s_prove_partials with that shard "
                "(asked for %zu of %zu)", pk->shard_index, pk->shard_count, pk->scheme, shard.index, shard.count);
  size_t wlo, whi, hlo, hhi;
  shard_range(w.n, shard, wlo, whi);
  if (sliced && eval) { hlo = pk->e_lo; hhi = pk->e_lo + pk->n_e; }
  else if (sliced) {
    hlo = std::min(pk->h_lo, nh);
    hhi = std::min(pk->h_lo + pk->n_h, nh);
  } else shard_range(nh, shard, hlo, hhi);
  const size_t held_lo = eval ? pk->e_lo : pk->h_lo;
  const size_t wbase = wlo - pk->w_lo, hbase = hlo - std::min(held_lo, hlo);
  if (wait_inputs) {
    hipEvent_t start;
    GS_HIP(hipEventCreateWithFlags(&start, hipEventDisableTiming));
    GS_HIP(hipEventRecord(start, c.main_stream));
    for (auto a : c.aux_stream) GS_HIP(hipStreamWaitEvent(a, start, 0));
    GS_HIP(hipEventDestroy(start));
  }
  int cw = 0, ch = 0;
  const int ng = pk->n_g1w, bg = pk->b_g1;
  KeyArray& harr = eval ? pk->h_eval : pk->h;
  const size_t n_harr = eval ? pk->n_e : pk->n_h;
  std::vector<BaseTable*> stamps;
  std::vector<TableRef> refs_w;
  for (int i = 0; i < ng; ++i) {
// ... 32 lines not shown
      uint32_t nb = 0;
      const uint32_t* list = term_list_range(pk->b_index, pk->b_index_host, wbase, nterms_w, nb);
      build_plan(c, 2 * Ctx::kSlots + parity, w.p + wlo * 8, nb, plan_b, {{1, true}, {1, false}}, cw, !tab_w, list, (uint32_t)wbase);
      st.tplanb->stop();
      GS_HIP(hipEventRecord(st.planb, c.stream));
    }
    st.tplanw = std::make_shared<PhaseTimer>(c.stream);
    build_plan(c, 0 + 2 * parity, w.p + wlo * 8, (uint32_t)nterms_w, plan_w,
               st.split_b ? std::vector<LaunchShape>{{ng - 1, false}} : std::vector<LaunchShape>{{1, true}, {ng, false}}, cw, !tab_w);
    st.tplanw->stop();
    GS_HIP(hipEventRecord(st.planw, c.stream));
  }
  auto enqueue_acc_w = [&] {
    StreamScope sc(c, c.main_stream);
    GS_HIP(hipStreamWaitEvent(c.stream, st.split_b ? st.planb : st.planw, 0));
    msm_enqueue_g2(c, st.split_b ? plan_b : plan_w, {base_w(pk->g2w)}, ws + pk->ws_g2, pin + 1, st.pend_g2w, ps.tail_g2);
    GS_HIP(hipEventRecord(st.done_g2, ps.tail_g2));
    std::vector<MsmBase> group;
    for (int i = 0; i < ng; ++i) if (!(st.split_b && i == bg)) group.push_back(base_w(pk->g1w[i]));
    if (st.split_b) {
      msm_enqueue_g1(c, plan_b, {base_w(pk->g1w[bg])}, ws + pk->ws_b, 3 * Ctx::kSlots + parity, st.pend_g1b, ps.tail_g1);
      GS_HIP(hipEventRecord(st.done_g1b, ps.tail_g1));
      GS_HIP(hipStreamWaitEvent(c.stream, st.planw, 0));
    }
    msm_enqueue_g1(c, plan_w, group, ws + 0, pin + 0, st.pend_g1w, ps.tail_g1);
    GS_HIP(hipEventRecord(st.done_g1w, ps.tail_g1));
  };
  auto enqueue_poly = [&] {
    StreamScope sc(c, ps.poly);
    if (px.host && px.n && px.host_stream) {
      staged_h2d(c, const_cast<uint32_t*>(px.p), px.host, px.n * 32, px.host_stream);
      if (host_stage_mode() == 1) GS_HIP(hipStreamSynchronize(px.host_stream));
      else {
        GS_HIP(hipEventRecord(px.host_done, px.host_stream));
        GS_HIP(hipStreamWaitEvent(c.stream, px.host_done, 0));
      }
    } else if (px.host && px.n && pipelined) {
      staged_h2d(c, const_cast<uint32_t*>(px.p), px.host, px.n * 32, c.stream);
    } else if (px.host && px.n) {
      PhaseTimer th(c.stream);
      staged_h2d(c, const_cast<uint32_t*>(px.p), px.host, px.n * 32, c.stream);
      th.stop();
      c.timing.h2d_ms += th.ms();
    }
    st.tpoly = std::make_shared<PhaseTimer>(c.stream);
    bool have_hx = false;
    if (px.hv_slice) have_hx = true;
    else if (eval) {
      px.produce_hv(c, hxbuf.as<uint32_t>(), c.bad_dev.as<uint32_t>() + parity);
      GS_HIP(hipMemcpyAsync(c.bad_host + parity, c.bad_dev.as<uint32_t>() + parity, 4, hipMemcpyDeviceToHost, c.stream));
      st.bad_host = c.bad_host + parity;
      have_hx = true;
    }
    if (!have_hx && px.produce_hx && nh) have_hx = px.produce_hx(c, hxbuf.as<uint32_t>());
    if (!have_hx) {
      if (px.produce) px.produce(c);
      if (nh) poly_quotient_dev(c, pk->z, px.p, px.n, hxbuf.as<uint32_t>());
    }
    st.tpoly->stop();
    st.tplanh = std::make_shared<PhaseTimer>(c.stream);
    build_plan(c, 1 + 2 * parity, px.hv_slice ? px.hv_slice : hxbuf.as<uint32_t>() + hlo * 8, (uint32_t)(hhi - hlo), plan_h, {{1, false}}, ch, !tab_h);
    st.tplanh->stop();
    GS_HIP(hipEventRecord(st.planh, c.stream));
  };
  if (ps.poly_first) { enqueue_poly(); enqueue_acc_w(); } else { enqueue_acc_w(); enqueue_poly(); }
  {
    StreamScope sc(c, c.main_stream);
    GS_HIP(hipStreamWaitEvent(c.stream, st.planh, 0));
    msm_enqueue_g1(c, plan_h, {MsmBase{&harr.table, hbase, harr.pts.as<uint32_t>(), n_harr}}, ws + pk->ws_h, pin + 2, st.pend_h,
                   pipelined ? ps.tail_g1 : nullptr);
    GS_HIP(hipEventRecord(st.done_h, pipelined ? ps.tail_g1 : c.main_stream));
  }
  st.total->stop();
  GS_HIP(hipEventRecord(st.done_main, c.main_stream));
  return GS_OK;
}

static double host_now_ms() {
  return std::chrono::duration<double, std::milli>(std::chrono::steady_clock::now().time_since_epoch()).count();
}
static bool host_trace() { static const bool on = run_flag("GS_HOST_TRACE"); return on; }

int proof_collect(Ctx& c, ProofInFlight& st, ProofSums& sums) {
  const double t0 = host_trace() ? host_now_ms() : 0;
  double t1 = 0;
  std::vector<G1Xyzz> g1h;
  std::vector<G2Xyzz> g2w;
  {
    GS_HIP(hipEventSynchronize(st.done_g2));
    auto f2 = std::async(std::launch::async, [&] { msm_finish_g2(c, st.pend_g2w, g2w); });
    struct Join { std::future<void>& f; ~Join() { if (f.valid()) f.wait(); } } j2{f2};
    GS_HIP(hipEventSynchronize(st.done_g1w));
    auto f1 = std::async(std::launch::async, [&] {
      msm_finish_g1(c, st.pend_g1w, sums.g1w);
      if (st.split_b) {
        std::vector<G1Xyzz> g1b;
        msm_finish_g1(c, st.pend_g1b, g1b);
        sums.g1w.insert(sums.g1w.begin() + st.pk->b_g1, g1b[0]);
      }
      if (st.on_g1w) st.on_g1w(sums.g1w);
    });
    Join j1{f1};
    GS_HIP(hipEventSynchronize(st.done_h));
    t1 = host_trace() ? host_now_ms() : 0;
    msm_finish_g1(c, st.pend_h, g1h);
    f2.get(); f1.get();
  }
  GS_HIP(hipEventSynchronize(st.done_main));
  if (host_trace()) fprintf(stderr, "[gs host] collect: wait %.3f ms, fold %.3f ms\n", t1 - t0, host_now_ms() - t1);
  msm_book_timing(c, st.pend_g1w); msm_book_timing(c, st.pend_g2w); msm_book_timing(c, st.pend_h);
  if (st.split_b) { msm_book_timing(c, st.pend_g1b); c.timing.plan_ms += st.tplanb->ms(); }
  c.timing.poly_ms += st.tpoly->ms();
  c.timing.plan_ms += st.tplanw->ms() + st.tplanh->ms();
  c.timing.total_ms += st.total->ms();
  if (st.in.th2d) c.timing.h2d_ms += st.in.th2d->ms();
  sums.g2w = g2w[0]; sums.h = g1h[0];
  if (st.bad_host && *st.bad_host != 0) return kRetryExact;
  return GS_OK;
}

int proof_sums_blocking(Ctx& c, ProverKey* pk, DevScalars w, DevScalars px, const Shard& shard, ProofSums& sums,
                        std::function<void(const std::vector<G1Xyzz>&)> on_g1w = nullptr) {
  for (;;) {
    const double t0 = host_trace() ? host_now_ms() : 0;
    ProofInFlight st;
    st.on_g1w = std::move(on_g1w);
    on_g1w = nullptr;
    int rc = proof_enqueue(c, pk, w, px, shard, c.blocking_slot(), true, false, st);
    if (rc != GS_OK) return rc;
    const double t1 = host_trace() ? host_now_ms() : 0;
    rc = proof_collect(c, st, sums);
    if (host_trace()) fprintf(stderr, "[gs host] prove: enqueue %.3f ms, collect %.3f ms (entered at %.3f)\n", t1 - t0, host_now_ms() - t1, t0);
    if (rc != kRetryExact) return rc;
    px.produce_hv = nullptr;
    c.timing.fallbacks += 1;
  }
}

struct GrothTailPre {
  std::future<G2Xyzz> sdelta2;
  std::future<G1Xyzz> sdelta;
  G1Xyzz rdelta, rsdelta;
};
static void groth16_tail_pre(GrothPkObj* pk, const uint64_t r[4], const uint64_t s[4], GrothTailPre& pre) {
  std::call_once(pk->fixed_once, [pk] { pk->delta_fixed.build(pk->delta); pk->delta2_fixed.build(pk->delta2); });
  uint64_t s_copy[4] = {s[0], s[1], s[2], s[3]};
  pre.sdelta2 = std::async(std::launch::async, [pk, s_copy] { return pk->delta2_fixed.mul(s_copy); });
  pre.sdelta = std::async(std::launch::deferred, [pk, s_copy] { return pk->delta_fixed.mul(s_copy); });
  pre.rdelta = pk->delta_fixed.mul(r);
  uint64_t rs[4];
  fr_mul_words(r, s, rs);
  pre.rsdelta = pk->delta_fixed.mul(rs);
}
struct GrothTail {
  GrothPkObj* pk = nullptr;
  uint64_t r[4] = {0, 0, 0, 0}, s[4] = {0, 0, 0, 0};
  GrothTailPre pre;
  std::future<void> fpre;
  bool early_done = false;
  G1Xyzz piA, piB1, sA, rB;
  void start(GrothPkObj* key, const uint64_t r_[4], const uint64_t s_[4]) {
    pk = key;
    memcpy(r, r_, 32); memcpy(s, s_, 32);
    fpre = std::async(std::launch::async, [this] { groth16_tail_pre(pk, r, s, pre); });
  }
  void products(const std::vector<G1Xyzz>& g1w) {
    piA = g1w[GrothPkObj::kAt];
    xyzz_madd(piA, pk->alpha);
    xyzz_add(piA, pre.rdelta);
    piB1 = g1w[GrothPkObj::kBacGamma1];
    xyzz_madd(piB1, pk->beta);
    xyzz_add(piB1, pre.sdelta.get());
    const G1Xyzz b1 = piB1;
    const uint64_t* rr = r;
    auto f_rB = std::async(std::launch::async, [b1, rr] { return g1_mul_scalar(b1, rr); });
    sA = g1_mul_scalar(piA, s);
    rB = f_rB.get();
  }
  void early(const std::vector<G1Xyzz>& g1w) {
    fpre.wait();
    products(g1w);
    early_done = true;
  }
  void finish(const ProofSums& sums, uint64_t out_proof[32], int inf[3]) {
    if (fpre.valid()) fpre.get();
    if (!early_done) products(sums.g1w);
// ... 156 lines not shown
  if (nw != o->m) return fail(GS_ERR_SHAPE, "len(w) = %zu but the system has %zu variables", nw, o->m);
  if (chk.need_z && pk->nz == 0) return fail(GS_ERR_SHAPE, "the key has no Z");
  reset_timing(c);
  const uint32_t* wdev = w ? w->buf.as<uint32_t>() : upload_tmp(c, prove_state(c).up_w, w_host, nw);
  const bool eval = c.eval_basis && !(chk.eval_full_key_only && pk->shard_count != 1) && pk->n_eval == o->n && hx_shape(o->n, pk->nz);
  dw = DevScalars{wdev, nw};
  dp = witness_scalars_blocking(c, o, wdev, pk->nz, eval);
  return GS_OK;
}

struct TicketRequest {
  const char* fn;
  Kind kind;
  gs_handle hpk, hr1cs;
  bool witness;
  gs_handle hw, hpx;
  const uint64_t* w_host; size_t nw;
  const uint64_t* px_host; size_t npx;
  uint64_t* ticket;
  bool null_extra;
  bool ticket_with_handles;
  bool refuse_slice;
  bool need_z;
};
int begin_ticket(Ctx& c, const TicketRequest& q, const std::function<std::unique_ptr<ProofInFlight>(ProverKey*)>& make) {
  const bool host = q.w_host != nullptr || q.px_host != nullptr;
  ProverKey* pk = c.get<ProverKey>(q.hpk, q.kind);
  R1csObj* o = q.witness ? c.get<R1csObj>(q.hr1cs, Kind::R1cs) : nullptr;
  Scalars* w = host ? nullptr : c.get<Scalars>(q.hw, Kind::Scalars);
  Scalars* px = host || q.witness ? nullptr : c.get<Scalars>(q.hpx, Kind::Scalars);
  const bool bad_handle = !pk || (q.witness && !o) || (!host && (!w || (!q.witness && !px)));
  if (q.ticket_with_handles) {
    if (bad_handle || !q.ticket) return fail(GS_ERR_ARG, "%s: bad handle or null ticket", q.fn);
  } else if (bad_handle) return fail(GS_ERR_ARG, "%s: bad handle", q.fn);
  if (q.null_extra || !q.ticket || (host && !q.witness && ((q.nw && !q.w_host) || (q.npx && !q.px_host)))) return fail(GS_ERR_ARG, "null argument");
  if (host && !q.witness && (q.nw >= (1ull << 31) || q.npx >= (1ull << 31))) return fail(GS_ERR_ARG, "%s: too many scalars", q.fn);
  const size_t nw = host ? q.nw : w->n;
  if (q.witness && nw != o->m) return fail(GS_ERR_SHAPE, "len(w) = %zu but the system has %zu variables", nw, o->m);
  if ((host || q.witness) && nw != pk->nvars) return fail(GS_ERR_SHAPE, "len(w) = %zu but the key has %zu variables", nw, pk->nvars);
  if (q.refuse_slice && pk->shard_count != 1) return fail(GS_ERR_ARG, "%s: the key is a slice", q.fn);
  if (q.need_z && pk->nz == 0) return fail(GS_ERR_SHAPE, "the key has no Z");
  const int parity = c.free_parity();
  if (parity < 0) return fail(GS_ERR_BUSY, "%s: three operations are already outstanding; call gs_%s_prove_end first", q.fn, pk->scheme);
  std::unique_ptr<ProofInFlight> st = make(pk);
  st->pk = pk;
  st->keep = {c.share<Object>(q.hpk, q.kind)};
  if (q.witness) st->keep.push_back(c.share<Object>(q.hr1cs, Kind::R1cs));
  if (w) st->keep.push_back(c.share<Object>(q.hw, Kind::Scalars));
  if (px) st->keep.push_back(c.share<Object>(q.hpx, Kind::Scalars));
  const double h0 = host_trace() ? host_now_ms() : 0;
  const DevScalars dw = host ? stage_slot_w(c, parity, q.w_host, nw, st->in, !q.witness) : resident(w);
  const double h1 = host_trace() ? host_now_ms() : 0;
  DevScalars dp;
  if (!q.witness) dp = host ? slot_px_from_host(c, parity, q.px_host, q.npx, st->in) : resident(px);
  else {
    const bool eval = c.eval_basis && pk->n_eval == o->n && hx_shape(o->n, pk->nz);
    const uint32_t* wdev = dw.p;
    const size_t nz = pk->nz;
    dp = witness_scalars(o, wdev, nz, eval, [o, parity](Ctx& cc) { return exact_px_buffer(cc, o, parity); });
    if (!eval) {
      dp.p = exact_px_buffer(c, o, parity);
    } else {
      dp.produce_hx = nullptr; dp.produce = nullptr;
      st->exact_route = [pk, o, wdev, nw, nz](Ctx& cc, ProofSums& sums) {
        return proof_sums_blocking(cc, pk, DevScalars{wdev, nw}, witness_scalars_blocking(cc, o, wdev, nz, false), Shard{}, sums);
      };
    }
  }
  const double h2 = host_trace() ? host_now_ms() : 0;
  const int rc = proof_enqueue(c, pk, dw, dp, Shard{}, parity, false, true, *st);
  if (rc != GS_OK) return rc;
  if (host_trace()) fprintf(stderr, "[gs host] begin: stage w %.3f ms, stage px %.3f ms, enqueue %.3f ms\n", h1 - h0, h2 - h1, host_now_ms() - h2);
  if (st->in.th2d) st->in.th2d->stop();
  mark_ticket_reads(st->streams, w, px);
  st->ticket = c.new_ticket();
  *q.ticket = st->ticket;
  c.inflight[parity] = std::move(st);
  return GS_OK;
}
int collect_ticket(Ctx& c, ProofInFlight& st, ProofSums& sums) {
  reset_timing(c);
  int rc = proof_collect(c, st, sums);
  if (rc == kRetryExact && st.exact_route) { c.timing.fallbacks += 1; rc = st.exact_route(c, sums); }
  return rc;
}

static size_t scan_finite_terms(Ctx& c, const uint32_t* g1_pts, const uint32_t* g2_pts, size_t n, DevBuf& index_dev, std::vector<uint32_t>& index_host) {
  index_host.clear();
  index_dev.release();
  if (n == 0) return 0;
  const size_t words = (n + 31) / 32;
  DevBuf mask(words * 4);
  const size_t finite = finite_mask_dev(c, g1_pts, g2_pts, (uint32_t)n, mask.as<uint32_t>());
  if (finite == n) return finite;
  std::vector<uint32_t> bits(words);
  GS_HIP(hipMemcpyAsync(bits.data(), mask.p, words * 4, hipMemcpyDeviceToHost, c.stream));
  GS_HIP(hipStreamSynchronize(c.stream));
  index_host.reserve(finite);
  for (size_t wd = 0; wd < words; ++wd)
    for (uint32_t m = bits[wd]; m; m &= m - 1) index_host.push_back((uint32_t)(wd * 32 + (size_t)__builtin_ctz(m)));
  index_dev.alloc(std::max<size_t>(index_host.size(), 1) * 4);
  if (!index_host.empty()) {
    GS_HIP(hipMemcpyAsync(index_dev.p, index_host.data(), index_host.size() * 4, hipMemcpyHostToDevice, c.stream));
    GS_HIP(hipStreamSynchronize(c.stream));
  }
  return finite;
}

struct PkSrc { const DevBuf* buf; size_t lo; };
static void copy_slice(Ctx& c, Ctx& from, const PkSrc& s, size_t n, size_t words, DevBuf& dst) {
  dst.alloc(std::max<size_t>(n, 1) * words * 4);
  copy_between(c, dst.p, from, static_cast<const char*>(s.buf->p) + s.lo * words * 4, n * words * 4);
}
static void groth_force_public(Ctx& c, GrothPkObj& pk) {
  const size_t zero_hi = std::min(pk.npublic + 1, pk.w_lo + pk.n_w);
  if (zero_hi > pk.w_lo) force_infinity(c, pk.bacdelta(), zero_hi - pk.w_lo, kG1Aff);
}
static void set_shard(ProverKey& pk, size_t index, size_t count) {
  Shard sh; sh.index = index; sh.count = count;
  size_t lo, hi;
  pk.shard_index = index; pk.shard_count = count;
  shard_range(pk.nvars, sh, lo, hi);
  pk.w_lo = lo; pk.n_w = hi - lo;
  shard_range(pk.len_h, sh, lo, hi);
  pk.h_lo = lo; pk.n_h = hi - lo;
}
static void shard_extras(Ctx& c, GrothPkObj& pk, const GrothPkObj& full) {
  groth_force_public(c, pk);
  pk.alpha = full.alpha; pk.beta = full.beta; pk.delta = full.delta; pk.beta2 = full.beta2; pk.delta2 = full.delta2;
}
static void shard_extras(Ctx&, PinocchioPkObj&, const PinocchioPkObj&) {}

template <class Pk>
static int pk_shard_impl(Ctx& c, Ctx& from, const char* scheme, Pk* full, size_t shard_index, size_t shard_count, gs_handle* out) {
  if (!full || !out) return fail(GS_ERR_ARG, "gs_%s_pk_shard: bad proving-key handle or null output", scheme);
  if (full->shard_count != 1) return fail(GS_ERR_ARG, "gs_%s_pk_shard: the source key is itself a slice", scheme);
// ... 616 lines not shown
```

### go-snark-study_amd/csrc/runtime.h

```cpp
#pragma once
#include <hip/hip_runtime.h>
#include <stdint.h>

#include <atomic>
#include <condition_variable>
#include <cstdarg>
#include <cstdio>
#include <cstdlib>
#include <cstring>
#include <memory>
#include <mutex>
#include <string>
#include <unordered_map>
#include <vector>

#include "../../include/gosnark_hip.h"
#include "knobs.h"

namespace gs {

inline std::string& last_error_ref() {
  static thread_local std::string e;
  return e;
}
// ... 148 lines not shown
    { std::lock_guard<std::mutex> lk(m_); serving_ += 1; waiters = next_ != serving_; }
    if (waiters) cv_.notify_all();
  }
 private:
  std::mutex m_;
  std::condition_variable cv_;
  uint64_t next_ = 0, serving_ = 0;
};

struct Ctx {
  int logical = 0;
  int device = -1;
  bool ready = false;
  hipStream_t stream = nullptr;
  hipStream_t main_stream = nullptr;
  static constexpr int kAuxStreams = 3;
  hipStream_t aux_stream[kAuxStreams] = {nullptr, nullptr, nullptr};
#ifndef GS_MAX_IN_FLIGHT
#define GS_MAX_IN_FLIGHT 3
#endif
  static constexpr int kMaxInFlight = GS_MAX_IN_FLIGHT;
  static constexpr int kSlots = kMaxInFlight + 1;
  static constexpr int kBlockingSlot = kMaxInFlight;
  void* pinned[4 * kSlots] = {};
  DevBuf bad_dev;
  uint32_t* bad_host = nullptr;
  static constexpr int kStageBuffers = 4;
  static constexpr size_t kStageBytes = 64u << 20;
  void* stage[kStageBuffers] = {};
  hipEvent_t stage_ev[kStageBuffers] = {};
  hipStream_t copy_stream = nullptr;
  std::shared_ptr<InFlightBase> inflight[kMaxInFlight];
  unsigned tail_flip = 0;
  hipStream_t tail_stream(int which) { return aux_stream[((which ^ (int)(tail_flip & 1u)) & 1) ? 2 : 0]; }
  void next_tails(uint32_t n) {
    static const int mode = (int)run_knob("GS_TAIL_FLIP", 1, 0, 2);
    if (mode == 1 || (mode == 2 && n <= kTailFlipMaxTerms)) tail_flip ^= 1u;
  }
  static constexpr uint32_t kTailFlipMaxTerms = 1u << 18;
  uint64_t new_ticket() { return ((uint64_t)logical << kHandleDevShift) | ticket_counter()++; }
  int free_parity() const { for (int p = 0; p < kMaxInFlight; ++p) if (!inflight[p]) return p; return -1; }
  bool any_inflight() const { for (int p = 0; p < kMaxInFlight; ++p) if (inflight[p]) return true; return false; }
  int blocking_slot() const { const int p = free_parity(); return p >= 0 ? p : kBlockingSlot; }
  static constexpr size_t kPinnedBytes = 256 * 1024;
  FairMutex mu;
  std::unordered_map<uint64_t, std::shared_ptr<Object>> objs;
  uint64_t call_clock = 0;
  uint64_t evictions = 0;
  int window_bits = 0;
  int table_policy = 0;
  hipStream_t table_stream = nullptr;
  double build_balance = 0;
  bool eval_basis = true;
  gs_timing timing{};
  std::mutex timing_mu;
  static constexpr int kWsSets = 8 * kSlots;
  DevBuf ws_buckets[kWsSets], ws_chunks[kWsSets], ws_partials[kWsSets], ws_out[kWsSets];
  std::shared_ptr<void> msm_state, poly_state, prove_state;
  DevBuf ws_misc;
  DevBuf g1_pow2, g2_pow2;
  std::vector<hipEvent_t> events;

  template <class O> O* get(gs_handle h, Kind k) {
    auto it = objs.find(h);
    if (it == objs.end() || it->second->kind != k) return nullptr;
    return static_cast<O*>(it->second.get());
  }
  template <class O> std::shared_ptr<O> share(gs_handle h, Kind k) {
    auto it = objs.find(h);
    if (it == objs.end() || it->second->kind != k) return nullptr;
    return std::static_pointer_cast<O>(it->second);
  }
  gs_handle put(std::shared_ptr<Object> o) {
    uint64_t h = ((uint64_t)logical << kHandleDevShift) | handle_counter()++;
    objs[h] = std::move(o);
    return h;
  }
  template <class S> S& state(std::shared_ptr<void>& slot) {
    if (!slot) slot = std::make_shared<S>();
    return *static_cast<S*>(slot.get());
  }
  void drain() {
    if (main_stream) GS_HIP(hipStreamSynchronize(main_stream));
    for (auto a : aux_stream) if (a && a != main_stream) GS_HIP(hipStreamSynchronize(a));
  }
};

struct Registry {
  std::mutex mu;
  std::vector<std::shared_ptr<Ctx>> ctxs;
};
inline Registry& registry() {
  static Registry r;
  return r;
}
inline int& current_logical() {
  static thread_local int v = 0;
  return v;
}
inline std::shared_ptr<Ctx> ctx_ref(int logical, size_t* count = nullptr) {
  Registry& r = registry();
  std::lock_guard<std::mutex> lk(r.mu);
  if (count) *count = r.ctxs.size();
  if (logical < 0 || (size_t)logical >= r.ctxs.size()) return nullptr;
  return r.ctxs[logical];
}
// ... 130 lines not shown
```

### go/gosnarkhip/gosnarkhip.go

```go
package gosnarkhip

import "C"

import (
	"errors"
	"fmt"
	"math/big"
	"runtime"
	"unsafe"
)

type Handle uint64

type Error struct {
	Code int
	Msg  string
}

func (e *Error) Error() string { return fmt.Sprintf("gosnark-hip: status %d: %s", e.Code, e.Msg) }

func (e *Error) Busy() bool { return e.Code == -6 }

func call(f func() C.int) error {
	runtime.LockOSThread()
// ... 182 lines not shown
	out := make([]*big.Int, len(b)/4)
	for i := range out {
		out[i] = word(b[4*i:])
	}
	return out
}

func PolyMul(a, b []*big.Int, order *big.Int) ([]*big.Int, error) {
	if len(a) == 0 || len(b) == 0 {
		return nil, errors.New("gosnark-hip: PolyMul of an empty polynomial")
	}
	ab, err := Scalars(a, order)
	if err != nil {
		return nil, err
	}
	bb, err := Scalars(b, order)
	if err != nil {
		return nil, err
	}
	out := make([]uint64, 4*(len(a)+len(b)-1))
	err = call(func() C.int { return C.gs_poly_mul(ptr(ab), C.size_t(len(a)), ptr(bb), C.size_t(len(b)), ptr(out)) })
	runtime.KeepAlive(ab)
	runtime.KeepAlive(bb)
	if err != nil {
		return nil, err
	}
	return unpackScalars(out), nil
}

func PolyDiv(a, b []*big.Int, order *big.Int) (quo, rem []*big.Int, err error) {
	nq, nr := len(a)-len(b)+1, len(b)-1
	if nq < 1 || len(b) == 0 {
		return nil, nil, errors.New("gosnark-hip: PolyDiv needs len(a) >= len(b) >= 1")
	}
	ab, err := Scalars(a, order)
	if err != nil {
		return
	}
	bb, err := Scalars(b, order)
	if err != nil {
		return
	}
	qb := make([]uint64, 4*nq)
	rb := make([]uint64, 4*(nr+1))
	err = call(func() C.int { return C.gs_poly_div(ptr(ab), C.size_t(len(a)), ptr(bb), C.size_t(len(b)), ptr(qb), ptr(rb)) })
	runtime.KeepAlive(ab)
	runtime.KeepAlive(bb)
	if err != nil {
		return
	}
	return unpackScalars(qb), unpackScalars(rb[:4*nr]), nil
}

func LagrangeInterpolation(values []*big.Int, order *big.Int) ([]*big.Int, error) {
	vb, err := Scalars(values, order)
	if err != nil {
		return nil, err
	}
	out := make([]uint64, 4*len(values))
	err = call(func() C.int { return C.gs_lagrange_interpolation(ptr(vb), C.size_t(len(values)), ptr(out)) })
	runtime.KeepAlive(vb)
	if err != nil {
		return nil, err
	}
	return unpackScalars(out), nil
}

func PairingCheck(g1 [][3]*big.Int, g2 [][3][2]*big.Int) (bool, error) {
	if len(g1) != len(g2) {
		return false, errors.New("gosnark-hip: PairingCheck needs as many G1 as G2 points")
	}
	if len(g1) == 0 {
		return true, nil
	}
	a, err := G1Points(g1)
	if err != nil {
		return false, err
	}
	b, err := G2Points(g2)
	if err != nil {
		return false, err
	}
	var ok C.int
	err = call(func() C.int { return C.gs_pairing_check(ptr(a), ptr(b), C.size_t(len(g1)), &ok) })
	runtime.KeepAlive(a)
	runtime.KeepAlive(b)
	return ok == 1, err
}
```

### go/gosnarkhip/seams.go

```go
package gosnarkhip

import "C"

import (
	"errors"
	"math/big"
	"runtime"
	"unsafe"
)


func polyAddSub(a, b []*big.Int, order *big.Int, sub bool) ([]*big.Int, error) {
	n := len(a)
	if len(b) > n {
		n = len(b)
	}
	if n == 0 {
		return nil, nil
	}
	ab, err := Scalars(a, order)
	if err != nil {
		return nil, err
	}
	bb, err := Scalars(b, order)
// ... 288 lines not shown

func (k *Groth16Key) ProveWitnessBegin(q *R1CS, w Handle, r, s, order *big.Int) (Groth16Ticket, error) {
	rs, err := Scalars([]*big.Int{r, s}, order)
	if err != nil {
		return 0, err
	}
	var t C.uint64_t
	err = call(func() C.int {
		return C.gs_groth16_prove_witness_begin(C.gs_handle(k.h), C.gs_handle(q.h), C.gs_handle(w), ptr(rs[0:]), ptr(rs[4:]), &t)
	})
	runtime.KeepAlive(rs)
	return Groth16Ticket(t), err
}

func (k *PinocchioKey) ProveBegin(w, px Handle) (uint64, error) {
	var t C.uint64_t
	err := call(func() C.int { return C.gs_pinocchio_prove_begin(C.gs_handle(k.h), C.gs_handle(w), C.gs_handle(px), &t) })
	return uint64(t), err
}
func (k *PinocchioKey) ProveWitnessBegin(q *R1CS, w Handle) (uint64, error) {
	var t C.uint64_t
	err := call(func() C.int { return C.gs_pinocchio_prove_witness_begin(C.gs_handle(k.h), C.gs_handle(q.h), C.gs_handle(w), &t) })
	return uint64(t), err
}
func PinocchioProveEnd(ticket uint64) (PinocchioProof, error) {
	var out [72]uint64
	var inf [8]C.int
	err := call(func() C.int { return C.gs_pinocchio_prove_end(C.uint64_t(ticket), (*C.uint64_t)(unsafe.Pointer(&out[0])), &inf[0]) })
	if err != nil {
		return PinocchioProof{}, err
	}
	return pinocchioProofFromWords(out[:], inf[:]), nil
}

func (k *PinocchioKey) ProveResident(w, px Handle) (PinocchioProof, error) {
	var out [72]uint64
	var inf [8]C.int
	err := call(func() C.int {
		return C.gs_pinocchio_prove_resident(C.gs_handle(k.h), C.gs_handle(w), C.gs_handle(px), (*C.uint64_t)(unsafe.Pointer(&out[0])), &inf[0])
	})
	if err != nil {
		return PinocchioProof{}, err
	}
	return pinocchioProofFromWords(out[:], inf[:]), nil
}

func SetWindowBits(c int) error { return call(func() C.int { return C.gs_set_window_bits(C.int(c)) }) }
func SetEvalBasisRoute(on bool) error {
	v := C.int(0)
	if on {
		v = 1
	}
	return call(func() C.int { return C.gs_set_eval_basis(v) })
}
func VerifySetStrict(on bool) {
	v := C.int(0)
	if on {
		v = 1
	}
	C.gs_verify_set_strict(v)
}


func Len(h Handle) (int, error) {
	var n C.size_t
	err := call(func() C.int { return C.gs_len(C.gs_handle(h), &n) })
	return int(n), err
}

func CurrentDevice() int { return int(C.gs_get_device()) }

func DownloadG1(h Handle, n int) ([][3]*big.Int, error) {
	buf := make([]uint64, 12*n)
	if err := call(func() C.int { return C.gs_g1_download(C.gs_handle(h), ptr(buf), C.size_t(n)) }); err != nil {
		return nil, err
	}
	out := make([][3]*big.Int, n)
	for i := range out {
		out[i] = G1FromJacobian(buf[12*i:])
	}
	return out, nil
}
func DownloadG2(h Handle, n int) ([][3][2]*big.Int, error) {
	buf := make([]uint64, 24*n)
	if err := call(func() C.int { return C.gs_g2_download(C.gs_handle(h), ptr(buf), C.size_t(n)) }); err != nil {
		return nil, err
	}
	out := make([][3][2]*big.Int, n)
	for i := range out {
		out[i] = G2FromJacobian(buf[24*i:])
	}
	return out, nil
}

func FixedBaseG1(device int, scalars []*big.Int, order *big.Int) (Handle, error) {
	buf, err := Scalars(scalars, order)
	if err != nil {
		return 0, err
	}
	var h C.gs_handle
	err = onDevice(device, func() C.int { return C.gs_g1_fixed_base(ptr(buf), C.size_t(len(scalars)), &h) })
	runtime.KeepAlive(buf)
	return Handle(h), err
}
func FixedBaseG2(device int, scalars []*big.Int, order *big.Int) (Handle, error) {
	buf, err := Scalars(scalars, order)
	if err != nil {
		return 0, err
	}
	var h C.gs_handle
	err = onDevice(device, func() C.int { return C.gs_g2_fixed_base(ptr(buf), C.size_t(len(scalars)), &h) })
	runtime.KeepAlive(buf)
	return Handle(h), err
}

type Timing struct {
	TotalMs, PlanMs, AccumulateMs, ReduceMs, PolyMs, H2DMs, AccG1Ms, AccG2Ms float32
	AccG1Launches, AccG2Launches                                               uint32
	AccG1Terms, AccG2Terms, AccG1Adds, AccG2Adds                               uint64
	WindowBits, Fallbacks                                                      uint32
	PlanDigits, PlanEntries                                                    uint64
	HeavyBuckets                                                               uint32
}

func timingFromC(t *C.gs_timing) Timing {
	return Timing{float32(t.total_ms), float32(t.plan_ms), float32(t.accumulate_ms), float32(t.reduce_ms), float32(t.poly_ms), float32(t.h2d_ms),
		float32(t.acc_g1_ms), float32(t.acc_g2_ms), uint32(t.acc_g1_launches), uint32(t.acc_g2_launches), uint64(t.acc_g1_terms), uint64(t.acc_g2_terms),
		uint64(t.acc_g1_adds), uint64(t.acc_g2_adds), uint32(t.window_bits), uint32(t.fallbacks),
		uint64(t.plan_digits), uint64(t.plan_entries), uint32(t.heavy_buckets)}
}

func LastTiming() (Timing, error) {
	var t C.gs_timing
	err := call(func() C.int { return C.gs_last_timing(&t) })
	return timingFromC(&t), err
}
func DeviceTiming(device int) (Timing, error) {
	var t C.gs_timing
	err := call(func() C.int { return C.gs_device_timing(C.int(device), &t) })
	return timingFromC(&t), err
}

func CommInfo() (nranks, rank int, local bool, collectives uint64) {
	var n, r, l C.int
	var c C.uint64_t
	C.gs_comm_info(&n, &r, &l, &c)
	return int(n), int(r), l != 0, uint64(c)
}

func CommAllGather(send []byte, nranks int) ([]byte, error) {
	if len(send) == 0 {
		return nil, nil
	}
	recv := make([]byte, len(send)*nranks)
	err := call(func() C.int { return C.gs_comm_allgather(unsafe.Pointer(&send[0]), C.size_t(len(send)), unsafe.Pointer(&recv[0])) })
	runtime.KeepAlive(send)
	return recv, err
}

type Partials struct {
	Sums [48]uint64
	Inf  [5]int32
}

func partialsCall(f func(out *C.uint64_t, inf *C.int) C.int) (Partials, error) {
	var p Partials
	var inf [5]C.int
	err := call(func() C.int { return f((*C.uint64_t)(unsafe.Pointer(&p.Sums[0])), &inf[0]) })
	for i := range inf {
		p.Inf[i] = int32(inf[i])
	}
	return p, err
}

func (k *Groth16Key) ProvePartials(w, px Handle, shard, count int) (Partials, error) {
	return partialsCall(func(out *C.uint64_t, inf *C.int) C.int {
		return C.gs_groth16_prove_partials(C.gs_handle(k.h), C.gs_handle(w), C.gs_handle(px), C.size_t(shard), C.size_t(count), out, inf)
	})
}

func (k *Groth16Key) ProvePartialsValues(w, hvSlice Handle, shard, count int) (Partials, error) {
	return partialsCall(func(out *C.uint64_t, inf *C.int) C.int {
// ... 181 lines not shown
```

### include/gosnark_hip.h

```cpp
#ifndef GOSNARK_HIP_H
#define GOSNARK_HIP_H

#include <stddef.h>
#include <stdint.h>

#ifdef __cplusplus
extern "C" {
#endif
#if defined(__GNUC__)
#pragma GCC visibility push(default)
#endif

typedef uint64_t gs_handle;

typedef enum {
  GS_OK = 0,
  GS_ERR_NO_DEVICE = -1,
  GS_ERR_HIP = -2,
  GS_ERR_ARG = -3,
  GS_ERR_SHAPE = -4,
  GS_ERR_NOT_INIT = -5,
  GS_ERR_BUSY = -6
} gs_status;

int gs_init(const int* devices, int ndev);
void gs_shutdown(void);
int gs_device_count(void);
int gs_set_device(int logical_device);
int gs_get_device(void);
int gs_handle_device(gs_handle h);
const char* gs_last_error(void);
const char* gs_version(void);
int gs_free(gs_handle h);

int gs_g1_upload(const uint64_t* jacobian , size_t n, gs_handle* out);
int gs_g2_upload(const uint64_t* jacobian , size_t n, gs_handle* out);
int gs_len(gs_handle h, size_t* out);
int gs_g1_download(gs_handle bases, uint64_t* jacobian , size_t n);
int gs_g2_download(gs_handle bases, uint64_t* jacobian , size_t n);

int gs_g1_fixed_base(const uint64_t* scalars , size_t n, gs_handle* out);
int gs_g2_fixed_base(const uint64_t* scalars , size_t n, gs_handle* out);

int gs_scalars_upload(const uint64_t* scalars , size_t n, gs_handle* out);
int gs_scalars_download(gs_handle scalars, uint64_t* out , size_t n);
int gs_scalars_update(gs_handle scalars, const uint64_t* values , size_t n);

int gs_scalars_clone(gs_handle scalars, size_t off, size_t n, int target_device, gs_handle* out);
int gs_g1_clone(gs_handle bases, size_t off, size_t n, int target_device, gs_handle* out);
int gs_g2_clone(gs_handle bases, size_t off, size_t n, int target_device, gs_handle* out);

int gs_msm_g1(gs_handle bases, const uint64_t* scalars , size_t off, size_t n,
              uint64_t out_affine[8], int* is_inf);
int gs_msm_g2(gs_handle bases, const uint64_t* scalars , size_t off, size_t n,
              uint64_t out_affine[16], int* is_inf);
int gs_msm_g1_resident(gs_handle bases, size_t off, gs_handle scalars, size_t soff, size_t n,
                       uint64_t out_affine[8], int* is_inf);
int gs_msm_g2_resident(gs_handle bases, size_t off, gs_handle scalars, size_t soff, size_t n,
                       uint64_t out_affine[16], int* is_inf);
int gs_msm_g1_begin(gs_handle bases, size_t off, gs_handle scalars, size_t soff, size_t n, uint64_t* ticket);
int gs_msm_g2_begin(gs_handle bases, size_t off, gs_handle scalars, size_t soff, size_t n, uint64_t* ticket);
int gs_msm_end(uint64_t ticket, uint64_t* out_affine, int* is_inf);
int gs_g1_sum_affine(const uint64_t* pts , const int* inf, size_t n, uint64_t out_affine[8], int* is_inf);
int gs_g2_sum_affine(const uint64_t* pts , const int* inf, size_t n, uint64_t out_affine[16], int* is_inf);

int gs_poly_mul(const uint64_t* a, size_t na, const uint64_t* b, size_t nb, uint64_t* out);
int gs_poly_div(const uint64_t* a, size_t na, const uint64_t* b, size_t nb, uint64_t* quo, uint64_t* rem);
int gs_poly_add(const uint64_t* a, size_t na, const uint64_t* b, size_t nb, uint64_t* out);
int gs_poly_sub(const uint64_t* a, size_t na, const uint64_t* b, size_t nb, uint64_t* out);
int gs_poly_eval(const uint64_t* v, size_t n, const uint64_t x[4], uint64_t out[4]);
int gs_lagrange_interpolation(const uint64_t* values, size_t n, uint64_t* coeffs);
int gs_zpoly(size_t deg, uint64_t* out);
int gs_r1cs_to_px(size_t n, size_t m,
                  const uint32_t* a_rowptr, const uint32_t* a_col, const uint64_t* a_val,
                  const uint32_t* b_rowptr, const uint32_t* b_col, const uint64_t* b_val,
                  const uint32_t* c_rowptr, const uint32_t* c_col, const uint64_t* c_val,
                  const uint64_t* w, uint64_t* ax, uint64_t* bx, uint64_t* cx, uint64_t* px);

int gs_r1cs_upload(size_t n, size_t m,
                   const uint32_t* a_rowptr, const uint32_t* a_col, const uint64_t* a_val,
                   const uint32_t* b_rowptr, const uint32_t* b_col, const uint64_t* b_val,
                   const uint32_t* c_rowptr, const uint32_t* c_col, const uint64_t* c_val, gs_handle* out);
int gs_r1cs_px(gs_handle r1cs, gs_handle w, gs_handle* px_inout);

int gs_groth16_pk_create(gs_handle g1_at, gs_handle g1_bacgamma, gs_handle g2_bacgamma,
                         gs_handle bacdelta, gs_handle powers_tau_delta,
                         const uint64_t g1_alpha[12], const uint64_t g1_beta[12], const uint64_t g1_delta[12],
                         const uint64_t g2_beta[24], const uint64_t g2_delta[24],
                         const uint64_t* z, size_t nz, size_t nvars, size_t npublic, gs_handle* out);
int gs_groth16_prove(gs_handle pk, const uint64_t* w, size_t nw, const uint64_t* px, size_t npx,
                     const uint64_t r[4], const uint64_t s[4], uint64_t out_proof[32], int inf[3]);
int gs_groth16_prove_resident(gs_handle pk, gs_handle w, gs_handle px,
                              const uint64_t r[4], const uint64_t s[4], uint64_t out_proof[32], int inf[3]);

int gs_groth16_prove_r1cs(gs_handle pk, gs_handle r1cs, gs_handle w, gs_handle* px_inout, const uint64_t r[4], const uint64_t s[4],
                          uint64_t out_proof[32], int inf[3]);

int gs_groth16_prove_witness(gs_handle pk, gs_handle r1cs, gs_handle w, const uint64_t r[4], const uint64_t s[4],
                             uint64_t out_proof[32], int inf[3]);
int gs_groth16_pk_set_eval(gs_handle pk, gs_handle bases);
int gs_pk_eval_count(gs_handle pk, size_t* count);
int gs_groth16_prove_witness_begin(gs_handle pk, gs_handle r1cs, gs_handle w, const uint64_t r[4], const uint64_t s[4], uint64_t* ticket);

int gs_groth16_prove_begin(gs_handle pk, gs_handle w, gs_handle px, const uint64_t r[4], const uint64_t s[4], uint64_t* ticket);
int gs_groth16_prove_end(uint64_t ticket, uint64_t out_proof[32], int inf[3]);
int gs_groth16_prove_host_begin(gs_handle pk, const uint64_t* w, size_t nw, const uint64_t* px, size_t npx, const uint64_t r[4], const uint64_t s[4],
                                uint64_t* ticket);
int gs_groth16_prove_witness_host_begin(gs_handle pk, gs_handle r1cs, const uint64_t* w, size_t nw, const uint64_t r[4], const uint64_t s[4],
                                        uint64_t* ticket);
int gs_groth16_prove_witness_host(gs_handle pk, gs_handle r1cs, const uint64_t* w, size_t nw, const uint64_t r[4], const uint64_t s[4],
                                  uint64_t out_proof[32], int inf[3]);
int gs_ticket_cancel(uint64_t ticket);

int gs_groth16_prove_partials(gs_handle pk, gs_handle w, gs_handle px, size_t shard_index, size_t shard_count,
                              uint64_t out_sums[48], int inf[5]);
int gs_groth16_pk_create_shard(gs_handle g1_at, gs_handle g1_bacgamma, gs_handle g2_bacgamma, gs_handle bacdelta, gs_handle ptd,
                               const uint64_t g1_alpha[12], const uint64_t g1_beta[12], const uint64_t g1_delta[12],
                               const uint64_t g2_beta[24], const uint64_t g2_delta[24], const uint64_t* z, size_t nz,
                               size_t nvars, size_t npublic, size_t nptd_total, size_t shard_index, size_t shard_count,
                               gs_handle* out);
// ... 40 lines not shown
int gs_msm_g1_multi(const gs_handle* bases, const gs_handle* scalars, int ndev, uint64_t out_affine[8], int* is_inf, int* used_rccl);
int gs_msm_g2_multi(const gs_handle* bases, const gs_handle* scalars, int ndev, uint64_t out_affine[16], int* is_inf, int* used_rccl);
int gs_groth16_prove_multi(const gs_handle* pk, const gs_handle* w, const gs_handle* px, int ndev, const uint64_t r[4], const uint64_t s[4],
                           uint64_t out_proof[32], int inf[3], int* used_rccl);
int gs_groth16_prove_sharded(gs_handle pk, gs_handle w, gs_handle px, const uint64_t r[4], const uint64_t s[4], uint64_t out_proof[32], int inf[3]);
int gs_groth16_witness_values(gs_handle pk, gs_handle r1cs, gs_handle w, gs_handle* hv_inout, uint32_t* violated);
int gs_groth16_prove_partials_values(gs_handle pk, gs_handle w, gs_handle hv_slice, size_t shard_index, size_t shard_count,
                                     uint64_t out_sums[48], int inf[5]);
int gs_groth16_partials_values_begin(gs_handle pk, gs_handle w, gs_handle hv_slice, size_t shard_index, size_t shard_count, uint64_t* ticket);
int gs_groth16_partials_end(uint64_t ticket, uint64_t out_sums[48], int inf[5]);
int gs_groth16_prove_multi_values(const gs_handle* pk, const gs_handle* w, const gs_handle* hv_slices, int ndev, const uint64_t r[4], const uint64_t s[4],
                                  uint64_t out_proof[32], int inf[3], int* used_rccl);
int gs_groth16_prove_sharded_values(gs_handle pk, gs_handle w, gs_handle hv_slice, const uint64_t r[4], const uint64_t s[4], uint64_t out_proof[32], int inf[3]);
int gs_scalars_scatter(gs_handle full_on_root, size_t total, int root, gs_handle* slice_inout);
int gs_msm_g1_sharded(gs_handle bases, gs_handle scalars, uint64_t out_affine[8], int* is_inf);
int gs_msm_g2_sharded(gs_handle bases, gs_handle scalars, uint64_t out_affine[16], int* is_inf);
int gs_groth16_prove_batch(const gs_handle* pk_of_device, int ndev, const gs_handle* w, const gs_handle* px, size_t nproofs,
                           const uint64_t* r, const uint64_t* s, uint64_t* out_proofs, int* inf);

int gs_pinocchio_pk_shard(gs_handle full_pk, size_t shard_index, size_t shard_count, gs_handle* out);
int gs_pinocchio_pk_shard_to(gs_handle full_pk, size_t shard_index, size_t shard_count, int target_device, gs_handle* out);
int gs_pinocchio_prove_partials(gs_handle pk, gs_handle w, gs_handle px, size_t shard_index, size_t shard_count, uint64_t out_sums[72], int inf[8]);
int gs_pinocchio_witness_values(gs_handle pk, gs_handle r1cs, gs_handle w, gs_handle* hv_inout, uint32_t* violated);
int gs_pinocchio_prove_partials_values(gs_handle pk, gs_handle w, gs_handle hv_slice, size_t shard_index, size_t shard_count,
                                       uint64_t out_sums[72], int inf[8]);
int gs_pinocchio_combine(const uint64_t* sums , const int* inf_in , size_t n, uint64_t out_proof[72], int inf[8]);
int gs_pinocchio_prove_multi(const gs_handle* pk, const gs_handle* w, const gs_handle* px, int ndev, uint64_t out_proof[72], int inf[8], int* used_rccl);
int gs_pinocchio_prove_multi_values(const gs_handle* pk, const gs_handle* w, const gs_handle* hv_slices, int ndev, uint64_t out_proof[72], int inf[8],
                                    int* used_rccl);
int gs_pinocchio_prove_sharded(gs_handle pk, gs_handle w, gs_handle px, uint64_t out_proof[72], int inf[8]);
int gs_pinocchio_prove_sharded_values(gs_handle pk, gs_handle w, gs_handle hv_slice, uint64_t out_proof[72], int inf[8]);
int gs_pinocchio_prove_batch(const gs_handle* pk_of_device, int ndev, const gs_handle* w, const gs_handle* px, size_t nproofs,
                             uint64_t* out_proofs , int* inf );

typedef struct {
  float total_ms;
  float plan_ms;
  float accumulate_ms;
  float reduce_ms;
  float poly_ms;
  float h2d_ms;
  float acc_g1_ms;
  float acc_g2_ms;
  uint32_t acc_g1_launches, acc_g2_launches;
  uint64_t acc_g1_terms;
  uint64_t acc_g2_terms;
  uint64_t acc_g1_adds;
  uint64_t acc_g2_adds;
  uint32_t window_bits;
  uint32_t fallbacks;
  uint64_t plan_digits;
  uint64_t plan_entries;
  uint32_t heavy_buckets;
  uint32_t reserved;
} gs_timing;
int gs_last_timing(gs_timing* out);
int gs_device_timing(int logical_device, gs_timing* out);

typedef struct {
  uint64_t device_total_bytes, device_free_bytes;
  uint64_t library_bytes;
  uint64_t object_bytes;
  uint64_t table_bytes;
  uint64_t workspace_bytes;
  uint64_t objects;
  uint64_t evictions;
} gs_memory;
int gs_memory_query(gs_memory* out);
int gs_handle_bytes(gs_handle h, uint64_t* object_bytes, uint64_t* table_bytes);
int gs_release_tables(gs_handle h);
int gs_set_table_policy(int policy);
int gs_build_tables(gs_handle h, int route);
int gs_set_memory_limit(uint64_t bytes);
int gs_alloc_counters(uint64_t* allocs, uint64_t* frees);
int gs_abi_sizes(size_t* timing_bytes, size_t* memory_bytes);
int gs_trim(void);

int gs_set_window_bits(int c);
int gs_set_eval_basis(int enabled);

int gs_pairing(const uint64_t g1[12], const uint64_t g2[24], uint64_t out_fq12[48]);
int gs_pairing_check(const uint64_t* g1 , const uint64_t* g2 , size_t k, int* ok);
int gs_verify_set_strict(int on);

int gs_groth16_verify(const uint64_t vk_g1_alpha[12], const uint64_t vk_g2_beta[24], const uint64_t vk_g2_gamma[24],
                      const uint64_t vk_g2_delta[24], const uint64_t* vk_ic , size_t nic,
                      const uint64_t* public_signals , size_t npublic,
                      const uint64_t pi_a[12], const uint64_t pi_b[24], const uint64_t pi_c[12], int* ok);
int gs_pinocchio_verify(const uint64_t vka[24], const uint64_t vkb[12], const uint64_t vkc[24], const uint64_t g1kbg[12],
                        const uint64_t g2kbg[24], const uint64_t g2kg[24], const uint64_t vkz[24],
                        const uint64_t* vk_ic , size_t nic, const uint64_t* public_signals, size_t npublic,
                        const uint64_t* proof , int* ok, int* failed_check);

#if defined(__GNUC__)
#pragma GCC visibility pop
#endif
#ifdef __cplusplus
}
#endif
#endif
```

Before: 118.8 million.

## Add coset-based exact quotient for H(x) and packed 16-bit MSM sort counters

Adds a coset-evaluation route for computing the quotient polynomial H = P/Z. It checks the result probabilistically at a random point and falls back to the series division if the division is inexact; this is enabled by default in the prover. Separately, the MSM bucket sort gets a packed mode that stores two 16-bit histogram counters per LDS word. That lets all 2^16 buckets be handled in one range pass instead of several range blocks, at the cost of capping slice length at 65535. It also exposes new API entry points and a coset_retreats timing counter.

Result: slower. 116.0 million (-2.3%).

```diff
diff --git a/go-snark-study_amd/capi.py b/go-snark-study_amd/capi.py
--- a/go-snark-study_amd/capi.py
+++ b/go-snark-study_amd/capi.py
@@ -28,7 +28,7 @@
                    ("acc_g1_terms", ctypes.c_uint64), ("acc_g2_terms", ctypes.c_uint64),
                    ("acc_g1_adds", ctypes.c_uint64), ("acc_g2_adds", ctypes.c_uint64),
                    ("window_bits", ctypes.c_uint32), ("fallbacks", ctypes.c_uint32),
-                   ("plan_digits", ctypes.c_uint64), ("plan_entries", ctypes.c_uint64), ("heavy_buckets", ctypes.c_uint32), ("reserved", ctypes.c_uint32)])
+                   ("plan_digits", ctypes.c_uint64), ("plan_entries", ctypes.c_uint64), ("heavy_buckets", ctypes.c_uint32), ("coset_retreats", ctypes.c_uint32)])
 
 
 class Memory(ctypes.Structure):
@@ -64,6 +64,7 @@
     "gs_g2_sum_affine": [u64p, intp, ctypes.c_size_t, u64p, intp],
     "gs_poly_mul": [u64p, ctypes.c_size_t, u64p, ctypes.c_size_t, u64p],
     "gs_poly_div": [u64p, ctypes.c_size_t, u64p, ctypes.c_size_t, u64p, u64p],
+    "gs_poly_div_exact": [u64p, ctypes.c_size_t, u64p, ctypes.c_size_t, ctypes.c_uint64, u64p, u64p, ctypes.POINTER(ctypes.c_int)],
     "gs_poly_add": [u64p, ctypes.c_size_t, u64p, ctypes.c_size_t, u64p],
     "gs_poly_sub": [u64p, ctypes.c_size_t, u64p, ctypes.c_size_t, u64p],
     "gs_poly_eval": [u64p, ctypes.c_size_t, u64p, u64p],
@@ -154,6 +155,7 @@
     "gs_device_timing": [ctypes.c_int, ctypes.POINTER(Timing)],
     "gs_set_window_bits": [ctypes.c_int],
     "gs_set_eval_basis": [ctypes.c_int],
+    "gs_set_coset_quotient": [ctypes.c_int],
     "gs_memory_query": [ctypes.POINTER(Memory)],
     "gs_handle_bytes": [Handle, u64p, u64p],
     "gs_release_tables": [Handle],
@@ -479,6 +481,22 @@
     check(load_library().gs_set_eval_basis(1 if on else 0))
 
 
+def set_coset_quotient(on):
+    init()
+    check(load_library().gs_set_coset_quotient(1 if on else 0))
+
+
+def poly_div_exact(a_u64, b_u64, first_shift=0):
+    init()
+    a = np.ascontiguousarray(a_u64, dtype=np.uint64).reshape(-1, 4)
+    b = np.ascontiguousarray(b_u64, dtype=np.uint64).reshape(-1, 4)
+    quo = np.zeros((a.shape[0] - b.shape[0] + 1, 4), dtype=np.uint64)
+    shift = np.zeros(4, dtype=np.uint64)
+    inexact = ctypes.c_int(0)
+    check(load_library().gs_poly_div_exact(ptr64(a), a.shape[0], ptr64(b), b.shape[0], int(first_shift), ptr64(quo), ptr64(shift), ctypes.byref(inexact)))
+    return quo, sum(int(w) << (64 * i) for i, w in enumerate(shift)), bool(inexact.value)
+
+
 def set_window_bits(c):
     init()
     check(load_library().gs_set_window_bits(int(c)))
diff --git a/go-snark-study_amd/csrc/capi_msm.hip b/go-snark-study_amd/csrc/capi_msm.hip
--- a/go-snark-study_amd/csrc/capi_msm.hip
+++ b/go-snark-study_amd/csrc/capi_msm.hip
@@ -576,4 +576,15 @@
   return GS_OK;
 }
 
-}
+int gs_set_coset_quotient(int enabled) {
+  Registry& r = registry();
+  std::lock_guard<std::mutex> rl(r.mu);
+  if (r.ctxs.empty()) return fail(GS_ERR_NOT_INIT, "gs_init has not been called (or failed)");
+  for (auto& pc : r.ctxs) {
+    std::lock_guard<FairMutex> lk(pc->mu);
+    pc->coset_quotient = enabled != 0;
+  }
+  return GS_OK;
+}
+
+}
diff --git a/go-snark-study_amd/csrc/capi_poly.hip b/go-snark-study_amd/csrc/capi_poly.hip
--- a/go-snark-study_amd/csrc/capi_poly.hip
+++ b/go-snark-study_amd/csrc/capi_poly.hip
@@ -46,6 +46,29 @@
     }
     poly_canon_dev(c, q, nq, 0);
     download(c, quo, q, nq);
+    return GS_OK;
+  });
+}
+
+int gs_poly_div_exact(const uint64_t* a, size_t na, const uint64_t* b, size_t nb, uint64_t first_shift, uint64_t* quo, uint64_t shift_used[4], int* inexact) {
+  return guarded([&](Ctx& c) -> int {
+    if (!a || !b || !quo || !inexact || nb == 0 || na < nb) return fail(GS_ERR_ARG, "gs_poly_div_exact: need len(a) >= len(b) >= 1");
+    if (na >= (1ull << 27)) return fail(GS_ERR_ARG, "gs_poly_div_exact: dividend too large");
+    const uint32_t* da = upload_tmp(c, prove_state(c).up_a, a, na);
+    const uint32_t* db = upload_tmp(c, prove_state(c).up_b, b, nb);
+    Divisor d;
+    divisor_init(c, d, db, nb);
+    const size_t nq = na - nb + 1;
+    prove_state(c).up_o.ensure((nq + 1) * 32);
+    uint32_t* q = prove_state(c).up_o.as<uint32_t>();
+    uint32_t* verdict = q + nq * 8;
+    poly_quotient_coset_dev(c, d, da, na, q, verdict, first_shift);
+    poly_canon_dev(c, q, nq, 0);
+    uint32_t word = 0;
+    GS_HIP(hipMemcpyAsync(&word, verdict, 4, hipMemcpyDeviceToHost, c.stream));
+    download(c, quo, q, nq);
+    *inexact = word != 0;
+    if (shift_used) for (int i = 0; i < 4; ++i) shift_used[i] = d.shift[i];
     return GS_OK;
   });
 }
diff --git a/go-snark-study_amd/csrc/msm.hip b/go-snark-study_amd/csrc/msm.hip
--- a/go-snark-study_amd/csrc/msm.hip
+++ b/go-snark-study_amd/csrc/msm.hip
@@ -112,16 +112,22 @@
   const size_t ncount = (size_t)plan.nbuckets + 1;
   PlanParams pp{};
   pp.n = n; pp.c = plan.c; pp.W = plan.W; pp.B = plan.B;
-  pp.R = std::max<uint32_t>(1u, plan.B >> kRangeLog);
   pp.tf = table_free ? 1u : 0u;
+  static const bool packed_on = run_knob("GS_SORT_PACKED", 1, 0, 1) != 0;
+  const uint32_t packed_slices = (uint32_t)(((uint64_t)n + kPackedSliceMax - 1) / kPackedSliceMax);
+  const uint32_t packed_room = (uint32_t)((68ull << 20) / ((uint64_t)plan.B * plan.W * 4));
+  const bool packed = packed_on && !table_free && plan.B == (1u << kPackedLog) && packed_slices <= packed_room;
+  pp.R = packed ? 1u : std::max<uint32_t>(1u, plan.B >> kRangeLog);
   {
     const uint32_t want = std::max<uint32_t>(1u, 256u / (plan.W * pp.R));
     const uint32_t by_size = std::max<uint32_t>(1u, (n + 16383u) / 16384u);
     const uint32_t by_mem = std::max<uint32_t>(1u, (uint32_t)((64ull << 20) / ((uint64_t)plan.B * plan.W * 4)));
     pp.S = std::max<uint32_t>(1u, std::min(std::min<uint32_t>(16u, std::max<uint32_t>(want, 1u)), std::min(by_size, by_mem)));
     if (pp.R == 1 && !table_free) pp.S = std::max<uint32_t>(1u, std::min<uint32_t>(16u, by_size));
+    if (packed) pp.S = std::max(packed_slices, std::min(std::min(want, by_size), packed_room));
   }
   pp.slice = (n + pp.S - 1) / pp.S;
+  if (packed && pp.slice > kPackedSliceMax) throw HipError{hipErrorInvalidValue, "slice too long for 16-bit sort counters", __LINE__};
   pp.stride = (n + 63u) & ~63u;
   const bool wide = plan_partitions_first(plan.c);
   if (wide && term_index) throw HipError{hipErrorInvalidValue, "plans over a term list cannot be sorted partition-first (plan_partitions_first)", __LINE__};
@@ -139,11 +145,13 @@
   pb.chunk_bucket.ensure((size_t)plan.maxchunks * 4);
   pb.heavy_list.ensure((size_t)plan.nbuckets * 4);
   pb.counters.ensure(16);
-  const size_t lds = (size_t)std::min<uint32_t>(plan.B, kRangeBuckets) * 4;
+  const size_t lds = packed ? (size_t)(1u << kPackedLog) * 2 : (size_t)std::min<uint32_t>(plan.B, kRangeBuckets) * 4;
   static const int sort_block = (int)dev_knob("GS_SORT_BLOCK", kSortBlock, 64, kSortBlock, 64);
   if (!ms.lds_attr_set) {
-    GS_HIP(hipFuncSetAttribute(reinterpret_cast<const void*>(k_hist), hipFuncAttributeMaxDynamicSharedMemorySize, 128 * 1024));
-    GS_HIP(hipFuncSetAttribute(reinterpret_cast<const void*>(k_scatter), hipFuncAttributeMaxDynamicSharedMemorySize, 128 * 1024));
+    GS_HIP(hipFuncSetAttribute(reinterpret_cast<const void*>(k_hist<false>), hipFuncAttributeMaxDynamicSharedMemorySize, 128 * 1024));
+    GS_HIP(hipFuncSetAttribute(reinterpret_cast<const void*>(k_scatter<false>), hipFuncAttributeMaxDynamicSharedMemorySize, 128 * 1024));
+    GS_HIP(hipFuncSetAttribute(reinterpret_cast<const void*>(k_hist<true>), hipFuncAttributeMaxDynamicSharedMemorySize, 128 * 1024));
+    GS_HIP(hipFuncSetAttribute(reinterpret_cast<const void*>(k_scatter<true>), hipFuncAttributeMaxDynamicSharedMemorySize, 128 * 1024));
     GS_HIP(hipFuncSetAttribute(reinterpret_cast<const void*>(k_hist_part), hipFuncAttributeMaxDynamicSharedMemorySize, 128 * 1024));
     GS_HIP(hipFuncSetAttribute(reinterpret_cast<const void*>(k_scatter_part), hipFuncAttributeMaxDynamicSharedMemorySize, 128 * 1024));
     ms.lds_attr_set = true;
@@ -163,7 +171,8 @@
     hipLaunchKernelGGL(k_colscan, grid1(plan.B), dim3(256), 0, c.stream, pb.hist.as<uint32_t>(), pp, pb.totals.as<uint32_t>());
   } else if (n > 0) {
     hipLaunchKernelGGL(k_digits, grid1(n), dim3(256), 0, c.stream, scalars_dev, pp, pb.digits.as<digit_t>(), term_index, index_bias);
-    hipLaunchKernelGGL(k_hist, dim3(plan.W, pp.S, pp.R), dim3(sort_block), lds, c.stream, pb.digits.as<digit_t>(), pp, pb.hist.as<uint32_t>());
+    if (packed) hipLaunchKernelGGL(k_hist<true>, dim3(plan.W, pp.S, 1), dim3(sort_block), lds, c.stream, pb.digits.as<digit_t>(), pp, pb.hist.as<uint32_t>());
+    else hipLaunchKernelGGL(k_hist<false>, dim3(plan.W, pp.S, pp.R), dim3(sort_block), lds, c.stream, pb.digits.as<digit_t>(), pp, pb.hist.as<uint32_t>());
     if (table_free) hipLaunchKernelGGL(k_colscan_windows, grid1(plan.nbuckets), dim3(256), 0, c.stream, pb.hist.as<uint32_t>(), pp, pb.totals.as<uint32_t>());
     else hipLaunchKernelGGL(k_colscan, grid1(plan.B), dim3(256), 0, c.stream, pb.hist.as<uint32_t>(), pp, pb.totals.as<uint32_t>());
   } else {
@@ -173,7 +182,9 @@
   if (n > 0) {
     if (wide) hipLaunchKernelGGL(k_scatter_part, dim3(8 * pp.S * ((nparts + 7) / 8)), dim3(sort_block), lds, c.stream, pb.recs.as<uint2>(), part_base, pp,
                                  pb.hist.as<uint32_t>(), pb.offsets.as<uint32_t>(), pb.entries.as<uint32_t>());
-    else hipLaunchKernelGGL(k_scatter, dim3(plan.W, pp.S, pp.R), dim3(sort_block), lds, c.stream, pb.digits.as<digit_t>(), pp, pb.hist.as<uint32_t>(),
+    else if (packed) hipLaunchKernelGGL(k_scatter<true>, dim3(plan.W, pp.S, 1), dim3(sort_block), lds, c.stream, pb.digits.as<digit_t>(), pp, pb.hist.as<uint32_t>(),
+                                        pb.offsets.as<uint32_t>(), pb.entries.as<uint32_t>(), term_index, index_bias);
+    else hipLaunchKernelGGL(k_scatter<false>, dim3(plan.W, pp.S, pp.R), dim3(sort_block), lds, c.stream, pb.digits.as<digit_t>(), pp, pb.hist.as<uint32_t>(),
                             pb.offsets.as<uint32_t>(), pb.entries.as<uint32_t>(), term_index, index_bias);
     hipLaunchKernelGGL(k_chunk_map, grid1(plan.nbuckets), dim3(256), 0, c.stream, pb.offsets.as<uint32_t>(), plan.nbuckets, plan.chunk,
                        pb.chunk_bucket.as<uint32_t>(), pb.heavy_list.as<uint32_t>(), pb.counters.as<uint32_t>());
diff --git a/go-snark-study_amd/csrc/msm_kernels.h b/go-snark-study_amd/csrc/msm_kernels.h
--- a/go-snark-study_amd/csrc/msm_kernels.h
+++ b/go-snark-study_amd/csrc/msm_kernels.h
@@ -20,6 +20,8 @@
 };
 constexpr uint32_t kRangeLog = 15;
 constexpr uint32_t kRangeBuckets = 1u << kRangeLog;
+constexpr uint32_t kPackedLog = 16;
+constexpr uint32_t kPackedSliceMax = 0xffffu;
 
 GS_HD int32_t next_digit(const uint32_t (&k)[8], const PlanParams& pp, int w, uint32_t& carry) {
   uint32_t raw = scalar_bits(k, w * pp.c, pp.c) + carry;
@@ -62,12 +64,14 @@
 
 constexpr int kSortBlock = 1024;
 
+template <bool kPacked>
 __global__ void __launch_bounds__(kSortBlock) k_hist(const digit_t* __restrict__ digits, PlanParams pp, uint32_t* __restrict__ hist) {
   wave_priority<GS_PRIO_PLAN>();
   extern __shared__ uint32_t sh[];
   const uint32_t w = blockIdx.x, s = blockIdx.y, r = blockIdx.z;
-  const uint32_t nb = min(pp.B, kRangeBuckets), base = r << kRangeLog;
-  for (uint32_t b = threadIdx.x; b < nb; b += blockDim.x) sh[b] = 0;
+  const uint32_t nb = kPacked ? (1u << kPackedLog) : min(pp.B, kRangeBuckets), base = kPacked ? 0u : r << kRangeLog;
+  const uint32_t nwords = kPacked ? nb / 2 : nb;
+  for (uint32_t b = threadIdx.x; b < nwords; b += blockDim.x) sh[b] = 0;
   __syncthreads();
   const uint32_t lo = s * pp.slice, hi = min(pp.n, lo + pp.slice);
   const digit_t* row = digits + (size_t)w * pp.stride;
@@ -76,12 +80,13 @@
     const int32_t d = (int32_t)row[i] - zero;
     if (d != 0) {
       const uint32_t b = (uint32_t)(d < 0 ? -d : d) - 1u;
-      if ((b >> kRangeLog) == r) atomicAdd(&sh[b - base], 1u);
+      if (kPacked) atomicAdd(&sh[b >> 1], 1u << (16u * (b & 1u)));
+      else if ((b >> kRangeLog) == r) atomicAdd(&sh[b - base], 1u);
     }
   }
   __syncthreads();
   uint32_t* out = hist + ((size_t)w * pp.S + s) * pp.B + base;
-  for (uint32_t b = threadIdx.x; b < nb; b += blockDim.x) out[b] = sh[b];
+  for (uint32_t b = threadIdx.x; b < nb; b += blockDim.x) out[b] = kPacked ? (sh[b >> 1] >> (16u * (b & 1u))) & 0xffffu : sh[b];
 }
 
 __global__ void __launch_bounds__(256) k_colscan(uint32_t* __restrict__ hist, PlanParams pp, uint32_t* __restrict__ totals) {
@@ -106,16 +111,18 @@
   totals[i] = run;
 }
 
+template <bool kPacked>
 __global__ void __launch_bounds__(kSortBlock) k_scatter(const digit_t* __restrict__ digits, PlanParams pp, const uint32_t* __restrict__ hist,
                                                          const uint32_t* __restrict__ offsets, uint32_t* __restrict__ entries,
                                                          const uint32_t* __restrict__ term_index, uint32_t index_bias) {
   wave_priority<GS_PRIO_PLAN>();
   extern __shared__ uint32_t sh[];
   const uint32_t w = blockIdx.x, s = blockIdx.y, r = blockIdx.z;
-  const uint32_t nb = min(pp.B, kRangeBuckets), base = r << kRangeLog;
+  const uint32_t nb = kPacked ? (1u << kPackedLog) : min(pp.B, kRangeBuckets), base = kPacked ? 0u : r << kRangeLog;
   const uint32_t* pre = hist + ((size_t)w * pp.S + s) * pp.B + base;
   const uint32_t* off = offsets + (pp.tf ? (size_t)w * pp.B : (size_t)0);
-  for (uint32_t b = threadIdx.x; b < nb; b += blockDim.x) sh[b] = off[base + b] + pre[b];
+  if (kPacked) for (uint32_t b = threadIdx.x; b < nb / 2; b += blockDim.x) sh[b] = 0;
+  else for (uint32_t b = threadIdx.x; b < nb; b += blockDim.x) sh[b] = off[base + b] + pre[b];
   __syncthreads();
   const uint32_t lo = s * pp.slice, hi = min(pp.n, lo + pp.slice);
   const digit_t* row = digits + (size_t)w * pp.stride;
@@ -124,8 +131,12 @@
     const int32_t d = (int32_t)row[i] - zero;
     if (d != 0) {
       const uint32_t b = (uint32_t)(d < 0 ? -d : d) - 1u;
-      if ((b >> kRangeLog) == r) {
-        const uint32_t pos = atomicAdd(&sh[b - base], 1u);
+      if (kPacked || (b >> kRangeLog) == r) {
+        uint32_t pos;
+        if (kPacked) {
+          const uint32_t sft = 16u * (b & 1u);
+          pos = ((atomicAdd(&sh[b >> 1], 1u << sft) >> sft) & 0xffffu) + off[b] + pre[b];
+        } else pos = atomicAdd(&sh[b - base], 1u);
         const uint32_t id = term_index ? term_index[i] - index_bias : i;
         entries[pos] = id | (w << kWindowShift) | (d < 0 ? kSignBit : 0u);
       }
diff --git a/go-snark-study_amd/csrc/poly.h b/go-snark-study_amd/csrc/poly.h
--- a/go-snark-study_amd/csrc/poly.h
+++ b/go-snark-study_amd/csrc/poly.h
@@ -25,9 +25,18 @@
   int logn_spec = 0;
   size_t k_spec = 0;
   DevBuf inv_spec;
+  size_t k_coset = 0;
+  int logn_coset = 0;
+  uint64_t shift[4] = {0, 0, 0, 0};
+  DevBuf coset_in;
+  DevBuf coset_inv;
+  DevBuf coset_out;
+  DevBuf bz;
 };
 void divisor_init(Ctx& c, Divisor& d, const uint32_t* b_std_dev, size_t nb);
 void poly_quotient_dev(Ctx& c, Divisor& d, const uint32_t* a_std, size_t na, uint32_t* quo_std);
+
+void poly_quotient_coset_dev(Ctx& c, Divisor& d, const uint32_t* a_std, size_t na, uint32_t* quo_std, uint32_t* verdict_dev, uint64_t first_shift = 0);
 
 void zpoly_dev(Ctx& c, size_t deg, uint32_t* out_std);
 
diff --git a/go-snark-study_amd/csrc/poly.hip b/go-snark-study_amd/csrc/poly.hip
--- a/go-snark-study_amd/csrc/poly.hip
+++ b/go-snark-study_amd/csrc/poly.hip
@@ -1,6 +1,7 @@
 #include "poly.h"
 
 #include <algorithm>
+#include <random>
 #include <vector>
 
 #include "poly_kernels.h"
@@ -61,6 +62,11 @@
   HxTables hx[kHxSlots];
   uint64_t hx_clock = 0;
   DevBuf hx_conv, hx_hv, hx_g, hx_bad;
+  uint64_t check_z[4] = {0, 0, 0, 0};
+  bool have_check_z = false;
+  DevBuf check_zlow, check_zhigh;
+  size_t check_tiles = 0;
+  DevBuf check_partial, coset_flag;
 };
 static PolyState& poly_state(Ctx& c) { return c.state<PolyState>(c.poly_state); }
 
@@ -231,6 +237,7 @@
   d.k = 0;
   d.logn_spec = 0;
   d.k_spec = 0;
+  d.k_coset = 0;
 }
 
 static void divisor_ensure(Ctx& c, Divisor& d, size_t k) {
@@ -269,6 +276,125 @@
   poly_state(c).ws_b.ensure(k * 32);
   hipLaunchKernelGGL(k_copy_reversed, grid1(k), dim3(256), 0, c.stream, A, 0u, (uint32_t)k, poly_state(c).ws_b.as<uint32_t>(), (uint32_t)k);
   hipLaunchKernelGGL(k_pw_mul_const, grid1(k), dim3(256), 0, c.stream, poly_state(c).ws_b.as<uint32_t>(), inv_n_const(logn, 0), quo, (uint32_t)k);
+  GS_HIP(hipGetLastError());
+}
+
+static const uint64_t* check_point(Ctx& c) {
+  PolyState& ps = poly_state(c);
+  if (!ps.have_check_z) {
+    std::random_device rd;
+    for (int i = 0; i < 4; ++i) ps.check_z[i] = ((uint64_t)rd() << 32) | (uint64_t)rd();
+    ps.check_z[3] &= (1ull << 61) - 1;
+    ps.have_check_z = true;
+  }
+  return ps.check_z;
+}
+static void raw_words(const Fe<ModR, 2>& v, uint64_t out[4]);
+static void ensure_check_tables(Ctx& c, size_t ntiles) {
+  PolyState& ps = poly_state(c);
+  if (ntiles <= ps.check_tiles) return;
+  if (ps.check_tiles) {
+    GS_HIP(hipStreamSynchronize(c.stream));
+    if (c.aux_stream[1] && c.aux_stream[1] != c.stream) GS_HIP(hipStreamSynchronize(c.aux_stream[1]));
+  }
+  ntiles = std::max(ntiles, 2 * ps.check_tiles);
+  const uint64_t* z = check_point(c);
+  uint64_t one_m[4], zt[4] = {z[0], z[1], z[2], z[3]};
+  raw_words(relax<2>(fe_one<ModR>()), one_m);
+  for (int i = 0; i < 11; ++i) fr_mul_words(zt, zt, zt);
+  static_assert(kCheckTile == 2048 && kCheckBlock == 256, "power tables of the coset check");
+  ps.check_zlow.alloc((kCheckBlock + 1) * 32);
+  ps.check_zhigh.alloc(ntiles * 32);
+  ps.check_partial.alloc(2 * ntiles * 32);
+  scaled_powers_dev(c, z, one_m, kCheckBlock + 1, ps.check_zlow.as<uint32_t>());
+  scaled_powers_dev(c, zt, one_m, ntiles, ps.check_zhigh.as<uint32_t>());
+  GS_HIP(hipStreamSynchronize(c.stream));
+  ps.check_tiles = ntiles;
+}
+static void raw_words(const Fe<ModR, 2>& v, uint64_t out[4]) {
+  uint32_t w[8];
+  pack32<ModR>(canon(v), w);
+  for (int i = 0; i < 4; ++i) out[i] = (uint64_t)w[2 * i] | ((uint64_t)w[2 * i + 1] << 32);
+}
+static const uint64_t kCosetShifts[3][4] = {
+  {0x9e3779b97f4a7c15ull, 0xf39cc0605cedc834ull, 0x1082276bf3a27251ull, 0},
+  {0x6a09e667f3bcc908ull, 0xbb67ae8584caa73bull, 0x3c6ef372fe94f82bull, 0},
+  {0x243f6a8885a308d3ull, 0x13198a2e03707344ull, 0xa4093822299f31d0ull, 0},
+};
+
+static void coset_forward(Ctx& c, const uint32_t* a, size_t na, const uint32_t* gpow, int logN, uint32_t* out) {
+  Twiddles& tw = ensure_twiddles(c, logN);
+  bool first = true;
+  for (const NttPass& p : ntt_schedule((size_t)1 << logN, logN)) {
+    if (first) hipLaunchKernelGGL((k_ntt_pass<false, kNttLoadCoset>), dim3(p.ntiles), dim3(256), 0, c.stream, out, tw.fwd.as<uint32_t>(), tw.logn, p.s_lo, p.k, p.clog,
+                                  NttLoadAux{a, gpow, (uint32_t)na, (uint32_t)logN});
+    else hipLaunchKernelGGL((k_ntt_pass<false, kNttLoadPlain>), dim3(p.ntiles), dim3(256), 0, c.stream, out, tw.fwd.as<uint32_t>(), tw.logn, p.s_lo, p.k, p.clog, NttLoadAux{});
+    first = false;
+  }
+  GS_HIP(hipGetLastError());
+}
+
+static bool coset_tables(Ctx& c, Divisor& d, int logN, const uint64_t g[4]) {
+  PolyState& ps = poly_state(c);
+  const size_t N = (size_t)1 << logN;
+  uint64_t one_m[4], invn_m[4], ginv[4];
+  raw_words(relax<2>(fe_one<ModR>()), one_m);
+  raw_words(inv(fr_small_mont(1ull << logN)), invn_m);
+  fr_inv_words(g, ginv);
+  d.coset_in.alloc((N + 1) * 32);
+  d.coset_inv.alloc(N * 32);
+  d.coset_out.alloc(N * 32);
+  d.bz.alloc(32);
+  ps.coset_flag.ensure(4);
+  scaled_powers_dev(c, g, one_m, N + 1, d.coset_in.as<uint32_t>());
+  coset_forward(c, d.b_std.as<uint32_t>(), d.nb, d.coset_in.as<uint32_t>(), logN, d.coset_inv.as<uint32_t>());
+  GS_HIP(hipMemsetAsync(ps.coset_flag.p, 0, 4, c.stream));
+  hipLaunchKernelGGL(k_pw_inv, grid1(N), dim3(256), 0, c.stream, d.coset_inv.as<uint32_t>(), (uint32_t)N, ps.coset_flag.as<uint32_t>());
+  GS_HIP(hipGetLastError());
+  uint32_t zero = 0;
+  GS_HIP(hipMemcpyAsync(&zero, ps.coset_flag.p, 4, hipMemcpyDeviceToHost, c.stream));
+  GS_HIP(hipStreamSynchronize(c.stream));
+  if (zero) return false;
+  scaled_powers_dev(c, ginv, invn_m, N, d.coset_out.as<uint32_t>());
+  poly_eval_dev(c, d.b_std.as<uint32_t>(), d.nb, check_point(c), d.bz.as<uint32_t>());
+  poly_canon_dev(c, d.bz.as<uint32_t>(), 1, 1);
+  GS_HIP(hipStreamSynchronize(c.stream));
+  for (int i = 0; i < 4; ++i) d.shift[i] = g[i];
+  return true;
+}
+
+static void coset_ensure(Ctx& c, Divisor& d, size_t k, int logN, uint64_t first_shift) {
+  if (d.k_coset == k && d.logn_coset == logN && !first_shift) return;
+  if (d.k_coset) {
+    GS_HIP(hipStreamSynchronize(c.stream));
+    if (c.aux_stream[1] && c.aux_stream[1] != c.stream) GS_HIP(hipStreamSynchronize(c.aux_stream[1]));
+  }
+  d.k_coset = 0;
+  const uint64_t first[4] = {first_shift, 0, 0, 0};
+  bool ok = first_shift && coset_tables(c, d, logN, first);
+  for (const auto& g : kCosetShifts) if (!ok) ok = coset_tables(c, d, logN, g);
+  if (!ok) throw HipError{hipErrorInvalidValue, "no coset shift avoids the roots of the divisor", __LINE__};
+  d.k_coset = k;
+  d.logn_coset = logN;
+}
+
+void poly_quotient_coset_dev(Ctx& c, Divisor& d, const uint32_t* a, size_t na, uint32_t* quo, uint32_t* verdict_dev, uint64_t first_shift) {
+  if (na < d.nb) { GS_HIP(hipMemsetAsync(verdict_dev, 0, 4, c.stream)); return; }
+  const size_t k = na - d.nb + 1;
+  const int logN = std::max(1, ceil_log2(k));
+  const size_t N = (size_t)1 << logN;
+  coset_ensure(c, d, k, logN, first_shift);
+  PolyState& ps = poly_state(c);
+  const size_t ntiles = (na + kCheckTile - 1) / kCheckTile;
+  ensure_check_tables(c, ntiles);
+  ps.ws_a.ensure(N * 32);
+  uint32_t* A = ps.ws_a.as<uint32_t>();
+  coset_forward(c, a, na, d.coset_in.as<uint32_t>(), logN, A);
+  ntt_inverse_unscaled_of_product_n(c, A, N, logN, d.coset_inv.as<uint32_t>());
+  hipLaunchKernelGGL(k_pw_mul, grid1(k), dim3(256), 0, c.stream, A, d.coset_out.as<uint32_t>(), quo, (uint32_t)k);
+  hipLaunchKernelGGL(k_check_partials, dim3((unsigned)ntiles), dim3(kCheckBlock), 0, c.stream, a, (uint32_t)na, quo, (uint32_t)k, ps.check_zlow.as<uint32_t>(),
+                     ps.check_zhigh.as<uint32_t>(), ps.check_partial.as<uint32_t>());
+  hipLaunchKernelGGL(k_coset_verdict, dim3(1), dim3(kCheckBlock), 0, c.stream, ps.check_partial.as<uint32_t>(), (uint32_t)ntiles, d.bz.as<uint32_t>(), verdict_dev);
   GS_HIP(hipGetLastError());
 }
 
diff --git a/go-snark-study_amd/csrc/poly_kernels.h b/go-snark-study_amd/csrc/poly_kernels.h
--- a/go-snark-study_amd/csrc/poly_kernels.h
+++ b/go-snark-study_amd/csrc/poly_kernels.h
@@ -164,7 +164,7 @@
   ntt_dit_step<20, N>(x, w, true, lazy_out, trivial);
 }
 
-constexpr int kNttLoadPlain = 0, kNttLoadScaled = 1, kNttLoadWeighed = 2;
+constexpr int kNttLoadPlain = 0, kNttLoadScaled = 1, kNttLoadWeighed = 2, kNttLoadCoset = 3;
 struct NttLoadAux {
   const uint32_t* aux0;
   const uint32_t* aux1;
@@ -196,6 +196,17 @@
       const uint32_t j = (uint32_t)(gi & (((size_t)1 << aux.logN) - 1));
       if (j < aux.n) v = mul(load_fr(aux.aux0 + (vec * aux.n + j) * 8), load_fr(aux.aux1 + (size_t)j * 8));
       else v = fe_zero<ModR, 2>();
+    } else if constexpr (kLoad == kNttLoadCoset) {
+      const uint32_t j = (uint32_t)gi;
+      if (j < aux.n) {
+        uint32_t t = (aux.n - 1 - j) >> aux.logN;
+        Fr2 acc = reduce2(load_fr(aux.aux0 + ((size_t)j + ((size_t)t << aux.logN)) * 8));
+        if (t) {
+          const Fr6 gN = load_fr(aux.aux1 + ((size_t)1 << aux.logN) * 8);
+          while (t--) acc = reduce2(add(mul(acc, gN), load_fr(aux.aux0 + ((size_t)j + ((size_t)t << aux.logN)) * 8)));
+        }
+        v = mul(acc, load_fr(aux.aux1 + (size_t)j * 8));
+      } else v = fe_zero<ModR, 2>();
     } else if constexpr (kLoad == kNttLoadScaled) {
       v = mul(reduce2(load_fr(x + gi * 8)), load_fr(aux.aux0 + (gi & (((size_t)1 << aux.logN) - 1)) * 8));
     } else {
@@ -274,6 +285,64 @@
   if (i >= n) return;
   store_fr(out + (size_t)i * 8, mul(load_fr(a + (size_t)i * 8), load_fr(b + (size_t)i * 8)));
 }
+__global__ void __launch_bounds__(256) k_pw_inv(uint32_t* __restrict__ x, uint32_t n, uint32_t* __restrict__ zero) {
+  const uint32_t i = blockIdx.x * blockDim.x + threadIdx.x;
+  if (i >= n) return;
+  const Fr2 v = reduce2(load_fr(x + (size_t)i * 8));
+  if (is_zero(v)) atomicOr(zero, 1u);
+  Fe<ModR, 1> one;
+#pragma unroll
+  for (int l = 0; l < NL; ++l) one.l[l] = (l == 0) ? 1u : 0u;
+  store_fr(x + (size_t)i * 8, mul(inv(v), one));
+}
+constexpr int kCheckBlock = 256, kCheckPer = 8, kCheckTile = kCheckBlock * kCheckPer;
+__device__ __forceinline__ void check_block_sum(uint32_t* sh, Fr2& sa, Fr2& sq) {
+  const uint32_t t = threadIdx.x;
+#pragma unroll
+  for (int l = 0; l < NL; ++l) { sh[(2 * t) * NL + l] = sa.l[l]; sh[(2 * t + 1) * NL + l] = sq.l[l]; }
+  __syncthreads();
+  for (uint32_t half = kCheckBlock / 2; half >= 1; half >>= 1) {
+    if (t < half) {
+      Fr2 oa, oq;
+#pragma unroll
+      for (int l = 0; l < NL; ++l) { oa.l[l] = sh[(2 * (t + half)) * NL + l]; oq.l[l] = sh[(2 * (t + half) + 1) * NL + l]; }
+      sa = reduce2(add(sa, oa)); sq = reduce2(add(sq, oq));
+#pragma unroll
+      for (int l = 0; l < NL; ++l) { sh[(2 * t) * NL + l] = sa.l[l]; sh[(2 * t + 1) * NL + l] = sq.l[l]; }
+    }
+    __syncthreads();
+  }
+}
+__global__ void __launch_bounds__(kCheckBlock) k_check_partials(const uint32_t* __restrict__ a, uint32_t na, const uint32_t* __restrict__ q, uint32_t nq,
+                                                                 const uint32_t* __restrict__ zlow, const uint32_t* __restrict__ zhigh,
+                                                                 uint32_t* __restrict__ partial) {
+  wave_priority<GS_PRIO_POLY>();
+  __shared__ uint32_t sh[2 * kCheckBlock * NL];
+  const uint32_t b = blockIdx.x, t = threadIdx.x;
+  Fr2 p = mul(load_fr(zlow + (size_t)t * 8), load_fr(zhigh + (size_t)b * 8));
+  const Fr6 step = load_fr(zlow + (size_t)kCheckBlock * 8);
+  Fr2 sa = fe_zero<ModR, 2>(), sq = fe_zero<ModR, 2>();
+  for (int s = 0; s < kCheckPer; ++s) {
+    const uint32_t i = b * kCheckTile + s * kCheckBlock + t;
+    if (i < na) sa = reduce2(add(sa, mul(load_fr(a + (size_t)i * 8), p)));
+    if (i < nq) sq = reduce2(add(sq, mul(load_fr(q + (size_t)i * 8), p)));
+    p = mul(p, step);
+  }
+  check_block_sum(sh, sa, sq);
+  if (t == 0) { store_fr(partial + (size_t)(2 * b) * 8, sa); store_fr(partial + (size_t)(2 * b + 1) * 8, sq); }
+}
+__global__ void __launch_bounds__(kCheckBlock) k_coset_verdict(const uint32_t* __restrict__ partial, uint32_t ntiles, const uint32_t* __restrict__ bz,
+                                                                uint32_t* __restrict__ verdict) {
+  wave_priority<GS_PRIO_POLY>();
+  __shared__ uint32_t sh[2 * kCheckBlock * NL];
+  Fr2 sa = fe_zero<ModR, 2>(), sq = fe_zero<ModR, 2>();
+  for (uint32_t i = threadIdx.x; i < ntiles; i += kCheckBlock) {
+    sa = reduce2(add(sa, load_fr(partial + (size_t)(2 * i) * 8)));
+    sq = reduce2(add(sq, load_fr(partial + (size_t)(2 * i + 1) * 8)));
+  }
+  check_block_sum(sh, sa, sq);
+  if (threadIdx.x == 0) *verdict = is_zero(sub(sa, mul(sq, load_fr(bz)))) ? 0u : 1u;
+}
 __global__ void __launch_bounds__(256) k_pw_mul_const(const uint32_t* __restrict__ a, FrConst k, uint32_t* __restrict__ out, uint32_t n) {
   wave_priority<GS_PRIO_POLY>();
   const uint32_t i = blockIdx.x * blockDim.x + threadIdx.x;
diff --git a/go-snark-study_amd/csrc/prove.hip b/go-snark-study_amd/csrc/prove.hip
--- a/go-snark-study_amd/csrc/prove.hip
+++ b/go-snark-study_amd/csrc/prove.hip
@@ -47,11 +47,17 @@
   std::function<bool(Ctx&, uint32_t*)> produce_hx;
   std::function<void(Ctx&, uint32_t*, uint32_t*)> produce_hv;
   const uint32_t* hv_slice = nullptr;
+  bool series = false;
 };
 DevScalars resident(const Scalars* s) { return DevScalars{s->buf.as<uint32_t>(), s->n}; }
 
 size_t quotient_len(size_t npx, size_t nz) { return npx >= nz ? npx - nz + 1 : 0; }
 constexpr int kRetryExact = 1;
+
+static bool coset_quotient_on(const Ctx& c) {
+  static const bool env = run_knob("GS_COSET_QUOTIENT", 1, 0, 1) != 0;
+  return env && c.coset_quotient;
+}
 
 
 struct ProofSums {
@@ -124,6 +130,7 @@
   MsmPending pend_g1w, pend_g2w, pend_h;
   std::shared_ptr<PhaseTimer> tpoly, tplanw, tplanh;
   const uint32_t* bad_host = nullptr;
+  bool coset = false;
   std::function<int(Ctx&, ProofSums&)> exact_route;
   std::function<void(const std::vector<G1Xyzz>&)> on_g1w;
   ProofInFlight() {
@@ -262,10 +269,19 @@
       st.bad_host = c.bad_host + parity;
       have_hx = true;
     }
-    if (!have_hx && px.produce_hx && nh) have_hx = px.produce_hx(c, hxbuf.as<uint32_t>());
+    bool exact = !px.series && coset_quotient_on(c);
+    if (!have_hx && px.produce_hx && nh) {
+      have_hx = px.produce_hx(c, hxbuf.as<uint32_t>());
+      exact = exact && have_hx;
+    }
     if (!have_hx) {
       if (px.produce) px.produce(c);
-      if (nh) poly_quotient_dev(c, pk->z, px.p, px.n, hxbuf.as<uint32_t>());
+      if (nh && exact) {
+        poly_quotient_coset_dev(c, pk->z, px.p, px.n, hxbuf.as<uint32_t>(), c.bad_dev.as<uint32_t>() + parity);
+        GS_HIP(hipMemcpyAsync(c.bad_host + parity, c.bad_dev.as<uint32_t>() + parity, 4, hipMemcpyDeviceToHost, c.stream));
+        st.bad_host = c.bad_host + parity;
+        st.coset = true;
+      } else if (nh) poly_quotient_dev(c, pk->z, px.p, px.n, hxbuf.as<uint32_t>());
     }
     st.tpoly->stop();
     st.tplanh = std::make_shared<PhaseTimer>(c.stream);
@@ -342,6 +358,11 @@
     rc = proof_collect(c, st, sums);
     if (host_trace()) fprintf(stderr, "[gs host] prove: enqueue %.3f ms, collect %.3f ms (entered at %.3f)\n", t1 - t0, host_now_ms() - t1, t0);
     if (rc != kRetryExact) return rc;
+    if (st.coset) {
+      px.series = true;
+      c.timing.coset_retreats += 1;
+      continue;
+    }
     px.produce_hv = nullptr;
     c.timing.fallbacks += 1;
   }
@@ -604,8 +625,15 @@
   const DevScalars dw = host ? stage_slot_w(c, parity, q.w_host, nw, st->in, !q.witness) : resident(w);
   const double h1 = host_trace() ? host_now_ms() : 0;
   DevScalars dp;
-  if (!q.witness) dp = host ? slot_px_from_host(c, parity, q.px_host, q.npx, st->in) : resident(px);
-  else {
+  if (!q.witness) {
+    dp = host ? slot_px_from_host(c, parity, q.px_host, q.npx, st->in) : resident(px);
+    const DevScalars rw{dw.p, dw.n}, rp{dp.p, dp.n};
+    st->exact_route = [pk, rw, rp](Ctx& cc, ProofSums& sums) {
+      DevScalars series = rp;
+      series.series = true;
+      return proof_sums_blocking(cc, pk, rw, series, Shard{}, sums);
+    };
+  } else {
     const bool eval = c.eval_basis && pk->n_eval == o->n && hx_shape(o->n, pk->nz);
     const uint32_t* wdev = dw.p;
     const size_t nz = pk->nz;
@@ -633,7 +661,10 @@
 int collect_ticket(Ctx& c, ProofInFlight& st, ProofSums& sums) {
   reset_timing(c);
   int rc = proof_collect(c, st, sums);
-  if (rc == kRetryExact && st.exact_route) { c.timing.fallbacks += 1; rc = st.exact_route(c, sums); }
+  if (rc == kRetryExact && st.exact_route) {
+    if (st.coset) c.timing.coset_retreats += 1; else c.timing.fallbacks += 1;
+    rc = st.exact_route(c, sums);
+  }
   return rc;
 }
 
diff --git a/go-snark-study_amd/csrc/runtime.h b/go-snark-study_amd/csrc/runtime.h
--- a/go-snark-study_amd/csrc/runtime.h
+++ b/go-snark-study_amd/csrc/runtime.h
@@ -224,6 +224,7 @@
   hipStream_t table_stream = nullptr;
   double build_balance = 0;
   bool eval_basis = true;
+  bool coset_quotient = true;
   gs_timing timing{};
   std::mutex timing_mu;
   static constexpr int kWsSets = 8 * kSlots;
diff --git a/go/gosnarkhip/gosnarkhip.go b/go/gosnarkhip/gosnarkhip.go
--- a/go/gosnarkhip/gosnarkhip.go
+++ b/go/gosnarkhip/gosnarkhip.go
@@ -258,6 +258,33 @@
 	return unpackScalars(qb), unpackScalars(rb[:4*nr]), nil
 }
 
+func PolyDivExact(a, b []*big.Int, order *big.Int, firstShift uint64) (quo []*big.Int, inexact bool, err error) {
+	nq := len(a) - len(b) + 1
+	if nq < 1 || len(b) == 0 {
+		return nil, false, errors.New("gosnark-hip: PolyDivExact needs len(a) >= len(b) >= 1")
+	}
+	ab, err := Scalars(a, order)
+	if err != nil {
+		return
+	}
+	bb, err := Scalars(b, order)
+	if err != nil {
+		return
+	}
+	qb := make([]uint64, 4*nq)
+	shift := make([]uint64, 4)
+	var flag C.int
+	err = call(func() C.int {
+		return C.gs_poly_div_exact(ptr(ab), C.size_t(len(a)), ptr(bb), C.size_t(len(b)), C.uint64_t(firstShift), ptr(qb), ptr(shift), &flag)
+	})
+	runtime.KeepAlive(ab)
+	runtime.KeepAlive(bb)
+	if err != nil {
+		return
+	}
+	return unpackScalars(qb), flag != 0, nil
+}
+
 func LagrangeInterpolation(values []*big.Int, order *big.Int) ([]*big.Int, error) {
 	vb, err := Scalars(values, order)
 	if err != nil {
diff --git a/go/gosnarkhip/seams.go b/go/gosnarkhip/seams.go
--- a/go/gosnarkhip/seams.go
+++ b/go/gosnarkhip/seams.go
@@ -364,6 +364,14 @@
 		v = 1
 	}
 	return call(func() C.int { return C.gs_set_eval_basis(v) })
+}
+
+func SetCosetQuotient(on bool) error {
+	v := C.int(0)
+	if on {
+		v = 1
+	}
+	return call(func() C.int { return C.gs_set_coset_quotient(v) })
 }
 func VerifySetStrict(on bool) {
 	v := C.int(0)
@@ -433,13 +441,14 @@
 	WindowBits, Fallbacks                                                      uint32
 	PlanDigits, PlanEntries                                                    uint64
 	HeavyBuckets                                                               uint32
+	CosetRetreats                                                              uint32
 }
 
 func timingFromC(t *C.gs_timing) Timing {
 	return Timing{float32(t.total_ms), float32(t.plan_ms), float32(t.accumulate_ms), float32(t.reduce_ms), float32(t.poly_ms), float32(t.h2d_ms),
 		float32(t.acc_g1_ms), float32(t.acc_g2_ms), uint32(t.acc_g1_launches), uint32(t.acc_g2_launches), uint64(t.acc_g1_terms), uint64(t.acc_g2_terms),
 		uint64(t.acc_g1_adds), uint64(t.acc_g2_adds), uint32(t.window_bits), uint32(t.fallbacks),
-		uint64(t.plan_digits), uint64(t.plan_entries), uint32(t.heavy_buckets)}
+		uint64(t.plan_digits), uint64(t.plan_entries), uint32(t.heavy_buckets), uint32(t.coset_retreats)}
 }
 
 func LastTiming() (Timing, error) {
diff --git a/include/gosnark_hip.h b/include/gosnark_hip.h
--- a/include/gosnark_hip.h
+++ b/include/gosnark_hip.h
@@ -66,6 +66,7 @@
 
 int gs_poly_mul(const uint64_t* a, size_t na, const uint64_t* b, size_t nb, uint64_t* out);
 int gs_poly_div(const uint64_t* a, size_t na, const uint64_t* b, size_t nb, uint64_t* quo, uint64_t* rem);
+int gs_poly_div_exact(const uint64_t* a, size_t na, const uint64_t* b, size_t nb, uint64_t first_shift, uint64_t* quo, uint64_t shift_used[4], int* inexact);
 int gs_poly_add(const uint64_t* a, size_t na, const uint64_t* b, size_t nb, uint64_t* out);
 int gs_poly_sub(const uint64_t* a, size_t na, const uint64_t* b, size_t nb, uint64_t* out);
 int gs_poly_eval(const uint64_t* v, size_t n, const uint64_t x[4], uint64_t out[4]);
@@ -212,7 +213,7 @@
   uint64_t plan_digits;
   uint64_t plan_entries;
   uint32_t heavy_buckets;
-  uint32_t reserved;
+  uint32_t coset_retreats;
 } gs_timing;
 int gs_last_timing(gs_timing* out);
 int gs_device_timing(int logical_device, gs_timing* out);
@@ -238,6 +239,7 @@
 
 int gs_set_window_bits(int c);
 int gs_set_eval_basis(int enabled);
+int gs_set_coset_quotient(int enabled);
 
 int gs_pairing(const uint64_t g1[12], const uint64_t g2[24], uint64_t out_fq12[48]);
 int gs_pairing_check(const uint64_t* g1 , const uint64_t* g2 , size_t k, int* ok);
```
